# yukyeongleee/pggan

Hardware: AMD Instinct MI355X
Metric: images/sec (G+D+GP step) at 1024×1024 bs=4/GPU, 1/2/4/8 MI355X (higher is better)
Workload: dtype bf16; 1 GPU; C5 G+D+R1 train_step via ProgressiveGAN.train_step, stage 8 (1024x1024), batch 4/GPU, alpha 1.0, depths [512, 512, 512, 512, 256, 128, 64, 32, 16] (alpha = 1: the fade-in's zero-weight low-resolution branches elided, results bit-identical on the CPU double, PG_ENGINE=elide_zero_blend=0 computes them); global_batch=4, resolution=1024, parallelism=dp1

## Files before the change

### include/pggan_hip.h

```cpp
#ifndef PGGAN_HIP_H
#define PGGAN_HIP_H
#include <stddef.h>
#include <stdint.h>

#ifdef __cplusplus
extern "C" {
#endif

#define PG_OK 0
#define PG_ERR_ARG (-1)
#define PG_ERR_HIP (-2)
#define PG_ERR_UNSUPPORTED (-3)

#define PG_F32 0
#define PG_BF16 1

const char* pg_last_error(void);
int pg_version(void);

#define PG_SCRATCH_BYTES (4u << 20)
size_t pg_scratch_bytes(void);

#define PG_CONV_UPS_IN 1
#define PG_CONV_BIAS 2
#define PG_CONV_LRELU 4
#define PG_CONV_MASK 8
#define PG_CONV_POOL 16
#define PG_CONV_ACCUM 32
#define PG_CONV_PIXNORM 64
#define PG_CONV_Y2_BITS 128
#define PG_CONV_AUX_BITS 256
#define PG_CONV_X_BITS 512
#define PG_CONV_GZ_BITS 1024
#define PG_CONV_PNBWD 2048
#define PG_CONV_RGBW 4096
#define PG_CONV_RGBD 8192
#define PG_CONV_RGBO 16384

typedef struct {
  int B, H, W;
  int cin, cout;
  int x_cs, y_cs, aux_cs, y2_cs;
  int flags;
  float slope;
  float out_scale;
  int xb_cs;
} pg_conv_desc;

#define PG_PACK_FWD 0
#define PG_PACK_DGRAD 1
size_t pg_conv3x3_packed_elems(int mode, int cout, int cin);
int pg_conv3x3_pack(int dtype, int mode, int cout, int cin, const float* w_oihw, float scale,
                    void* wpk, void* stream);
typedef struct {
  const float* w;
  const float* bias;
  void* fwd;
  void* dgrad;
  float* bias_scaled;
  float scale;
  int cout, cin;
  int pad_;
} pg_pack_item;
int pg_conv3x3_pack_batch(int dtype, int n, const pg_pack_item* items, int max_tiles,
                          void* stream);
size_t pg_conv3x3_workspace_size(const pg_conv_desc* d);
int pg_conv3x3_fwd(int dtype, const pg_conv_desc* d, const void* x, const void* wpk,
                   const float* bias, const void* aux, void* y, void* y2, void* ws,
                   size_t ws_bytes, void* stream);
int pg_conv3x3_fwd_ex(int dtype, const pg_conv_desc* d, const void* x, const void* xbits,
                      const void* wpk, const float* bias, const void* aux, void* y, void* y2,
                      void* ws, size_t ws_bytes, void* stream);
int pg_conv3x3_rgbw(int dtype, const pg_conv_desc* d, const void* x, const void* wpk,
                    const void* aux, const float* img, float s, float* dw, float* db,
                    void* scratch, void* stream);
int pg_conv3x3_rgbd(int dtype, const pg_conv_desc* d, const void* x, const void* wpk,
                    const void* aux, const float* w_rgb, float f, float* gimg, float* norms,
                    float* dw, float s, void* scratch, void* stream);
int pg_conv3x3_rgbo(int dtype, const pg_conv_desc* d, const void* x, const void* wpk,
                    const float* bias, void* y, void* y2, const float* w_rgb, const float* b_rgb,
                    float c, float* img, void* stream);
int pg_conv3x3_supported(int dtype, const pg_conv_desc* d, size_t ws_bytes);
size_t pg_conv3x3_wgrad_workspace_size(int dtype, const pg_conv_desc* d);
int pg_conv3x3_wgrad(int dtype, const pg_conv_desc* d, const void* x, const void* gz, float scale,
                     float* dw, float* db, void* ws, size_t ws_bytes, void* stream);
int pg_conv3x3_wgrad_ex(int dtype, const pg_conv_desc* d, const void* x, const void* gz,
                        const void* gzbits, float scale, float* dw, float* db, void* ws,
                        size_t ws_bytes, void* stream);
int pg_bias_grad(int dtype, int npix, int C, int cs, const void* g, float scale, float* db,
                 void* scratch, void* stream);

int pg_pixnorm_fwd(int dtype, int npix, int C, int cs, const void* x, void* y, void* stream);
int pg_pixnorm_lrelu_bwd(int dtype, int npix, int C, int cs, const void* u, const void* gy,
                         float slope, int apply_mask, void* gz, void* stream);

int pg_pixnorm_lrelu_bwd_y(int dtype, int npix, int C, int cs, const void* y, const float* r,
                           const void* gy, float slope, void* gz, void* stream);
int pg_unpool_mask(int dtype, int B, int H, int W, int C, int g_cs, const void* g, int y_cs,
                   const void* y, float scale, float slope, int ups, int out_cs, void* out,
                   void* stream);
int pg_unpool_mask_bits(int dtype, int B, int H, int W, int C, int g_cs, const void* g,
                        const void* bits, float scale, float slope, int ups, int out_cs, void* out,
                        void* stream);
int pg_avgpool2(int dtype, int B, int H, int W, int C, int x_cs, const void* x, int y_cs, void* y,
                void* stream);
int pg_blend(int dtype, size_t n, float a, const void* x, float b, const void* y, void* out,
             void* stream);

int pg_rgb_out(int dtype, int B, int R, int C, int x_cs, const void* x, const float* w,
               const float* b, float c, int Cp, int xp_cs, const void* xp, const float* wp,
               const float* bp, float cp, float alpha, float* img, void* stream);
int pg_rgb_out_bwd(int dtype, int B, int R, int C, int x_cs, const void* x, const float* w,
                   float c, int Cp, int xp_cs, const void* xp, const float* wp, float cp,
                   float alpha, const float* gimg, void* gx, void* gxp, float* dw, float* db,
                   float* dwp, float* dbp, void* scratch, void* stream);
int pg_rgb_out_bwd_pn(int dtype, int B, int R, int C, int y_cs, const void* y, const float* r,
                      const float* w, float c, const float* gimg, float slope, int gz_cs, void* gz,
                      void* stream);
int pg_rgb_out_bwd_pn_wg(int dtype, int B, int R, int C, int y_cs, const void* y, const float* r,
                         const float* w, float c, const float* gimg, float slope, int gz_cs,
                         void* gz, float* dw, float* db, void* scratch, void* stream);
int pg_from_rgb(int dtype, int B, int R, int C, const float* img, int down, const float* w,
                const float* b, float c, float slope, const void* mask_y, int y_cs, void* y,
                void* stream);
int pg_from_rgb_bwd(int dtype, int B, int R, int C, const float* img, int down, const float* w,
                    float c, int gz_cs, const void* gz, float* gimg, float* dw, float* db,
                    void* scratch, void* stream);
typedef struct {
  const float* x0;
  const float* x1;
  const float* a;
  const float* c;
} pg_img_src;
int pg_from_rgb_src(int dtype, int B, int R, int C, const pg_img_src* img, int down, const float* w,
                    const float* b, float c, float slope, const void* mask_y, int y_cs, void* y,
                    void* stream);
int pg_from_rgb_bits(int dtype, int B, int R, int C, const pg_img_src* img, int down,
                     const float* w, const float* b, float c, float slope, const void* mask_bits,
                     int y_cs, void* y, void* ybits, void* stream);
int pg_from_rgb_bwd_src(int dtype, int B, int R, int C, const pg_img_src* img, int down,
                        const float* w, float c, int gz_cs, const void* gz, float* gimg,
                        int gimg_overwrite, float* norms, float* dw, float* db, void* scratch,
                        void* stream);
int pg_penalty_scale(int mode, int B, float* norms, float w, float* loss_out, float* scale,
                     void* stream);

int pg_img_fade(int B, int C, int R, const float* x, float alpha, float* out, void* stream);

#define PG_LIN_BIAS 1
#define PG_LIN_LRELU 2
#define PG_LIN_MASK 4
#define PG_LIN_IN_CHW 8
#define PG_LIN_OUT_CHW 16
#define PG_LIN_F32_IN 32
#define PG_LIN_F32_OUT 64
typedef struct {
  int B, K, N;
  int in_cs, out_cs;
  int flags;
  float scale, slope;
} pg_linear_desc;
int pg_linear_fwd(int dtype, const pg_linear_desc* d, const void* x, const float* w,
                  const float* b, const void* aux, void* y, void* stream);
int pg_linear_dgrad(int dtype, const pg_linear_desc* d, const void* gy, const float* w,
                    const void* aux, void* gx, void* stream);
size_t pg_linear_workspace_size(int dtype, const pg_linear_desc* d, int pass);
int pg_linear_fwd_ws(int dtype, const pg_linear_desc* d, const void* x, const float* w,
                     const float* b, const void* aux, void* y, void* ws, size_t ws_bytes,
                     void* stream);
int pg_linear_dgrad_ws(int dtype, const pg_linear_desc* d, const void* gy, const float* w,
                       const void* aux, void* gx, void* ws, size_t ws_bytes, void* stream);
// ... 67 lines not shown
```

### pggan_amd/_lib.py

```python
from __future__ import annotations

import ctypes
import os

import torch

PG_F32, PG_BF16 = 0, 1

CONV_UPS_IN, CONV_BIAS, CONV_LRELU, CONV_MASK, CONV_POOL, CONV_ACCUM = 1, 2, 4, 8, 16, 32
CONV_PIXNORM = 64
CONV_PNBWD = 2048
CONV_RGBW = 4096
CONV_RGBD = 8192
CONV_RGBO = 16384
CONV_Y2_BITS, CONV_AUX_BITS, CONV_X_BITS, CONV_GZ_BITS = 128, 256, 512, 1024
PACK_FWD, PACK_DGRAD = 0, 1
LIN_BIAS, LIN_LRELU, LIN_MASK, LIN_IN_CHW, LIN_OUT_CHW, LIN_F32_IN, LIN_F32_OUT = (
    1, 2, 4, 8, 16, 32, 64)

_HERE = os.path.dirname(os.path.abspath(__file__))
LIB_PATH = os.path.join(_HERE, "libpggan_hip.so")


class ConvDesc(ctypes.Structure):
    _fields_ = [(n, ctypes.c_int) for n in
                ("B", "H", "W", "cin", "cout", "x_cs", "y_cs", "aux_cs", "y2_cs", "flags")] + \
               [("slope", ctypes.c_float), ("out_scale", ctypes.c_float), ("xb_cs", ctypes.c_int)]


class PackItem(ctypes.Structure):
    _fields_ = [("w", ctypes.c_void_p), ("bias", ctypes.c_void_p), ("fwd", ctypes.c_void_p),
                ("dgrad", ctypes.c_void_p), ("bias_scaled", ctypes.c_void_p),
                ("scale", ctypes.c_float), ("cout", ctypes.c_int), ("cin", ctypes.c_int),
                ("pad_", ctypes.c_int)]


def _cinp(c):
    return (c + 7) // 8 * 8 if c <= 16 else (c + 31) // 32 * 32


class ImgMix:

    def __init__(self, x0, x1=None, a=None, c=None):
        self.x0, self.x1, self.a, self.c = x0, x1, a, c

    @property
    def shape(self):
        return self.x0.shape

    @property
    def device(self):
        return self.x0.device

    def materialize(self):
        if self.a is None:
            return self.x0
        v = self.a.view(-1, 1, 1, 1) * self.x0
        if self.x1 is not None:
            v = v + self.c.view(-1, 1, 1, 1) * self.x1
        return v


class ImgSrcDesc(ctypes.Structure):
    _fields_ = [("x0", ctypes.c_void_p), ("x1", ctypes.c_void_p), ("a", ctypes.c_void_p),
                ("c", ctypes.c_void_p)]


class LinearDesc(ctypes.Structure):
    _fields_ = [(n, ctypes.c_int) for n in ("B", "K", "N", "in_cs", "out_cs", "flags")] + \
               [("scale", ctypes.c_float), ("slope", ctypes.c_float)]


_lib = None
_SIDE_STREAMS = {}

_VP, _I, _F, _SZ, _U64 = ctypes.c_void_p, ctypes.c_int, ctypes.c_float, ctypes.c_size_t, ctypes.c_uint64
_SIGS = {
    "pg_version": ([], _I),
    "pg_scratch_bytes": ([], _SZ),
    "pg_conv3x3_packed_elems": ([_I, _I, _I], _SZ),
    "pg_conv3x3_pack": ([_I, _I, _I, _I, _VP, _F, _VP, _VP], _I),
    "pg_conv3x3_pack_batch": ([_I, _I, _VP, _I, _VP], _I),
    "pg_conv3x3_workspace_size": ([ctypes.POINTER(ConvDesc)], _SZ),
    "pg_conv3x3_fwd": ([_I, ctypes.POINTER(ConvDesc), _VP, _VP, _VP, _VP, _VP, _VP, _VP, _SZ, _VP],
                       _I),
    "pg_conv3x3_supported": ([_I, ctypes.POINTER(ConvDesc), _SZ], _I),
    "pg_conv3x3_rgbw": ([_I, ctypes.POINTER(ConvDesc), _VP, _VP, _VP, _VP, _F, _VP, _VP, _VP, _VP],
                        _I),
    "pg_conv3x3_rgbd": ([_I, ctypes.POINTER(ConvDesc), _VP, _VP, _VP, _VP, _F, _VP, _VP, _VP, _F,
                         _VP, _VP], _I),
    "pg_conv3x3_rgbo": ([_I, ctypes.POINTER(ConvDesc), _VP, _VP, _VP, _VP, _VP, _VP, _VP, _F, _VP,
                         _VP], _I),
    "pg_conv3x3_fwd_ex": ([_I, ctypes.POINTER(ConvDesc), _VP, _VP, _VP, _VP, _VP, _VP, _VP, _VP,
                           _SZ, _VP], _I),
    "pg_conv3x3_wgrad_ex": ([_I, ctypes.POINTER(ConvDesc), _VP, _VP, _VP, _F, _VP, _VP, _VP, _SZ,
                             _VP], _I),
    "pg_conv3x3_wgrad_workspace_size": ([_I, ctypes.POINTER(ConvDesc)], _SZ),
    "pg_conv3x3_wgrad": ([_I, ctypes.POINTER(ConvDesc), _VP, _VP, _F, _VP, _VP, _VP, _SZ, _VP],
                         _I),
    "pg_bias_grad": ([_I, _I, _I, _I, _VP, _F, _VP, _VP, _VP], _I),
    "pg_pixnorm_fwd": ([_I, _I, _I, _I, _VP, _VP, _VP], _I),
    "pg_pixnorm_lrelu_bwd": ([_I, _I, _I, _I, _VP, _VP, _F, _I, _VP, _VP], _I),
    "pg_pixnorm_lrelu_bwd_y": ([_I, _I, _I, _I, _VP, _VP, _VP, _F, _VP, _VP], _I),
    "pg_unpool_mask": ([_I, _I, _I, _I, _I, _I, _VP, _I, _VP, _F, _F, _I, _I, _VP, _VP], _I),
    "pg_unpool_mask_bits": ([_I, _I, _I, _I, _I, _I, _VP, _VP, _F, _F, _I, _I, _VP, _VP], _I),
    "pg_avgpool2": ([_I, _I, _I, _I, _I, _I, _VP, _I, _VP, _VP], _I),
    "pg_blend": ([_I, _SZ, _F, _VP, _F, _VP, _VP, _VP], _I),
    "pg_rgb_out": ([_I, _I, _I, _I, _I, _VP, _VP, _VP, _F, _I, _I, _VP, _VP, _VP, _F, _F, _VP,
                    _VP], _I),
    "pg_rgb_out_bwd": ([_I, _I, _I, _I, _I, _VP, _VP, _F, _I, _I, _VP, _VP, _F, _F, _VP, _VP,
                        _VP, _VP, _VP, _VP, _VP, _VP, _VP], _I),
    "pg_from_rgb": ([_I, _I, _I, _I, _VP, _I, _VP, _VP, _F, _F, _VP, _I, _VP, _VP], _I),
    "pg_from_rgb_bwd": ([_I, _I, _I, _I, _VP, _I, _VP, _F, _I, _VP, _VP, _VP, _VP, _VP, _VP], _I),
    "pg_img_fade": ([_I, _I, _I, _VP, _F, _VP, _VP], _I),
    "pg_from_rgb_src": ([_I, _I, _I, _I, ctypes.POINTER(ImgSrcDesc), _I, _VP, _VP, _F, _F, _VP, _I,
                         _VP, _VP], _I),
    "pg_rgb_out_bwd_pn": ([_I, _I, _I, _I, _I, _VP, _VP, _VP, _F, _VP, _F, _I, _VP, _VP], _I),
    "pg_rgb_out_bwd_pn_wg": ([_I, _I, _I, _I, _I, _VP, _VP, _VP, _F, _VP, _F, _I, _VP, _VP, _VP,
                              _VP, _VP], _I),
    "pg_from_rgb_bits": ([_I, _I, _I, _I, ctypes.POINTER(ImgSrcDesc), _I, _VP, _VP, _F, _F, _VP,
                          _I, _VP, _VP, _VP], _I),
    "pg_from_rgb_bwd_src": ([_I, _I, _I, _I, ctypes.POINTER(ImgSrcDesc), _I, _VP, _F, _I, _VP, _VP,
                             _I, _VP, _VP, _VP, _VP, _VP], _I),
    "pg_penalty_scale": ([_I, _I, _VP, _F, _VP, _VP, _VP], _I),
    "pg_linear_fwd": ([_I, ctypes.POINTER(LinearDesc), _VP, _VP, _VP, _VP, _VP, _VP], _I),
    "pg_linear_dgrad": ([_I, ctypes.POINTER(LinearDesc), _VP, _VP, _VP, _VP, _VP], _I),
    "pg_linear_wgrad": ([_I, ctypes.POINTER(LinearDesc), _VP, _VP, _VP, _VP, _VP], _I),
    "pg_linear_workspace_size": ([_I, ctypes.POINTER(LinearDesc), _I], _SZ),
    "pg_linear_fwd_ws": ([_I, ctypes.POINTER(LinearDesc), _VP, _VP, _VP, _VP, _VP, _VP, _SZ, _VP],
                         _I),
    "pg_linear_dgrad_ws": ([_I, ctypes.POINTER(LinearDesc), _VP, _VP, _VP, _VP, _VP, _SZ, _VP],
                           _I),
    "pg_mbstd_fwd": ([_I, _I, _I, _I, _I, _VP, _I, _VP, _VP], _I),
    "pg_mbstd_bwd": ([_I, _I, _I, _I, _I, _VP, _I, _VP, _VP, _VP], _I),
    "pg_mbstd_r1": ([_I, _I, _I, _I, _I, _VP, _VP, _I, _VP, _VP, _VP, _VP], _I),
    "pg_bce_loss": ([_I, _VP, _I, _F, _VP, _VP, _VP, _VP], _I),
    "pg_r1_penalty": ([_I, _SZ, _VP, _VP, _VP, _VP, _VP], _I),
    "pg_drift_loss": ([_I, _VP, _F, _VP, _VP, _VP], _I),
    "pg_gp_interp": ([_I, _SZ, _VP, _VP, _VP, _VP, _VP], _I),
    "pg_gp_penalty": ([_I, _SZ, _VP, _F, _VP, _VP, _VP, _VP, _VP], _I),
    "pg_mul_add": ([_SZ, _VP, _VP, _VP, _VP, _VP], _I),
    "pg_adam": ([_SZ, _VP, _VP, _VP, _VP, _F, _F, _F, _F, _I, _VP], _I),
    "pg_randn": ([_SZ, _U64, _U64, _VP, _VP], _I),
    "pg_randn_dev": ([_SZ, _U64, _VP, _VP, _VP], _I),
    "pg_adam_table_len": ([_F, _F, _F], _I),
    "pg_adam_table": ([_F, _F, _F, _I, _VP], _I),
    "pg_adam_dev": ([_SZ, _VP, _VP, _VP, _VP, _F, _F, _F, _VP, _I, _VP, _VP], _I),
    "pg_cast": ([_I, _I, _SZ, _VP, _VP, _VP], _I),
    "pg_augment_workspace_bytes": ([_I, _I, _I], _SZ),
    "pg_augment_u8": ([_I, _I, _I, _VP, _VP, _VP, _SZ, _VP, _VP], _I),
    "pg_step_plan_create": ([_I, _I, ctypes.POINTER(ctypes.c_int), _I, _I,
                             ctypes.POINTER(ctypes.c_void_p)], _I),
    "pg_step_plan_workspace_size": ([_VP], _SZ),
    "pg_step_plan_describe": ([_VP, ctypes.c_char_p, _SZ], _I),
    "pg_step_plan_destroy": ([_VP], None),
    "pg_event_create": ([_I, ctypes.POINTER(ctypes.c_void_p)], _I),
    "pg_event_record": ([_VP, _VP], _I),
    "pg_stream_wait_event": ([_VP, _VP], _I),
    "pg_event_elapsed_ms": ([_VP, _VP, ctypes.POINTER(ctypes.c_float)], _I),
    "pg_event_destroy": ([_VP], _I),
    "pg_fill_zero": ([_VP, _SZ, _VP], _I),
    "pg_copy": ([_VP, _VP, _SZ, _VP], _I),
    "pg_record_begin": ([], _I),
    "pg_record_end": ([ctypes.POINTER(ctypes.c_void_p)], _I),
    "pg_record_count": ([_VP], _I),
    "pg_replay": ([_VP], _I),
    "pg_record_destroy": ([_VP], None),
    "pg_stream_create": ([_I, ctypes.POINTER(ctypes.c_void_p)], _I),
    "pg_stream_destroy": ([_VP], _I),
}
SYMBOLS = ["pg_last_error"] + list(_SIGS)


def load_library(path: str = LIB_PATH):
    global _lib
    if _lib is not None:
        return _lib
    if not os.path.exists(path):
        raise RuntimeError(f"pggan_amd: HIP library not built: {path} (run __graft_entry__.build())")
    lib = ctypes.CDLL(path)
    lib.pg_last_error.argtypes = []
    lib.pg_last_error.restype = ctypes.c_char_p
# ... 152 lines not shown
    def conv_pack(self, mode, w, scale, out):
        self._cuda(w, out)
        cout, cin = w.shape[0], w.shape[1]
        self._chk(self.lib.pg_conv3x3_pack(self._dt(out), mode, cout, cin, _p(w), scale, _p(out),
                                           self._s()), "conv3x3_pack")

    def pack_table(self, entries):
        n = len(entries)
        arr = (PackItem * n)()
        mt = 1
        for i, (w, b, pf, pd, bs, sc) in enumerate(entries):
            self._cuda(w, b, pf, pd, bs)
            cout, cin = w.shape[0], w.shape[1]
            arr[i] = PackItem(_p(w), _p(b), _p(pf), _p(pd), _p(bs), float(sc), cout, cin, 0)
            O = max((cout + 15) // 16 * 16, _cinp(cout))
            C = max(_cinp(cin), (cin + 15) // 16 * 16)
            mt = max(mt, ((O + 31) // 32) * ((C + 31) // 32))
        raw = torch.frombuffer(bytearray(bytes(arr)), dtype=torch.uint8)
        return raw.to(entries[0][0].device), n, mt

    def conv_pack_batch(self, table):
        dev, n, mt = table
        self._cuda(dev)
        self._chk(self.lib.pg_conv3x3_pack_batch(self.dt, n, _p(dev), mt, self._s()),
                  "conv3x3_pack_batch")

    def conv3x3(self, x, wpk, y, *, B, H, W, cin, cout, flags, slope=0.2, out_scale=1.0,
                bias=None, aux=None, y2=None, ws=None, xbits=None):
        self._cuda(x, wpk, y, bias, aux, y2, ws, xbits)
        d = ConvDesc(B, H, W, cin, cout, x.shape[-1], y.shape[-1],
                     aux.shape[-1] if aux is not None else 0,
                     y2.shape[-1] if y2 is not None else 0, flags, slope, out_scale,
                     xbits.shape[-1] if xbits is not None else 0)
        wsb = ws.numel() * ws.element_size() if ws is not None else 0
        self._chk(self.lib.pg_conv3x3_fwd_ex(self._dt(y), ctypes.byref(d), _p(x), _p(xbits),
                                             _p(wpk), _p(bias), _p(aux), _p(y), _p(y2), _p(ws),
                                             wsb, self._s()),
                  "conv3x3_fwd")

    def conv3x3_rgbw(self, x, wpk, *, B, H, W, cin, cout, flags, aux, img, s, dw, db,
                     slope=0.2, out_scale=1.0):
        self._cuda(x, wpk, aux, img, dw, db)
        d = ConvDesc(B, H, W, cin, cout, x.shape[-1], cout, aux.shape[-1], 0,
                     flags | CONV_RGBW, slope, out_scale, 0)
        self._chk(self.lib.pg_conv3x3_rgbw(self._dt(x), ctypes.byref(d), _p(x), _p(wpk), _p(aux),
                                           _p(img), float(s), _p(dw), _p(db),
                                           self._scr(), self._s()),
                  "conv3x3_rgbw")

    def conv3x3_rgbo(self, x, wpk, y, *, B, H, W, cin, cout, flags, bias, w_rgb, b_rgb, c, img,
                     y2=None, slope=0.2):
        self._cuda(x, wpk, y, bias, y2, w_rgb, b_rgb, img)
        d = ConvDesc(B, H, W, cin, cout, x.shape[-1], y.shape[-1], 0,
                     y2.shape[-1] if y2 is not None else 0, flags | CONV_RGBO, slope, 1.0, 0)
        self._chk(self.lib.pg_conv3x3_rgbo(self._dt(y), ctypes.byref(d), _p(x), _p(wpk), _p(bias),
                                           _p(y), _p(y2), _p(w_rgb), _p(b_rgb), float(c), _p(img),
                                           self._s()),
                  "conv3x3_rgbo")

    def conv3x3_rgbd(self, x, wpk, *, B, H, W, cin, cout, flags, aux, w_rgb, f, gimg,
                     norms=None, dw=None, s=0.0, slope=0.2, out_scale=1.0):
        self._cuda(x, wpk, aux, w_rgb, gimg, norms, dw)
        d = ConvDesc(B, H, W, cin, cout, x.shape[-1], cout, aux.shape[-1], 0,
                     flags | CONV_RGBD, slope, out_scale, 0)
        self._chk(self.lib.pg_conv3x3_rgbd(self._dt(x), ctypes.byref(d), _p(x), _p(wpk), _p(aux),
                                           _p(w_rgb), float(f), _p(gimg), _p(norms), _p(dw),
                                           float(s), self._scr(), self._s()),
                  "conv3x3_rgbd")

    def conv_supported(self, *, B, H, W, cin, cout, flags, ws_bytes=0):
        if flags & CONV_GZ_BITS:
            return self.dt == PG_BF16 and H % 2 == 0 and W % 2 == 0 and cout % 8 == 0
        d = ConvDesc(B, H, W, cin, cout, 0, 0, 0, 0, flags, 0.2, 1.0, 0)
        return bool(self.lib.pg_conv3x3_supported(self.dt, ctypes.byref(d), ws_bytes))

    def conv_workspace_bytes(self, *, B, H, W, cin, cout):
        d = ConvDesc(B, H, W, cin, cout, 0, 0, 0, 0, 0, 0.0, 1.0, 0)
        return int(self.lib.pg_conv3x3_workspace_size(ctypes.byref(d)))

    def wgrad_workspace_bytes(self, *, B, H, W, cin, cout, ups=False):
        d = ConvDesc(B, H, W, cin, cout, 0, 0, 0, 0, CONV_UPS_IN if ups else 0, 0.0, 1.0, 0)
        return int(self.lib.pg_conv3x3_wgrad_workspace_size(self.dt, ctypes.byref(d)))

    def conv_wgrad(self, x, gz, dw, *, B, H, W, cin, cout, ups, scale, db=None, ws=None,
                   gzbits=None, slope=0.2):
        self._cuda(x, gz, dw, db, ws, gzbits)
        fl = (CONV_UPS_IN if ups else 0) | (CONV_GZ_BITS if gzbits is not None else 0)
        d = ConvDesc(B, H, W, cin, cout, x.shape[-1], gz.shape[-1], 0, 0, fl, slope, 1.0,
                     gzbits.shape[-1] if gzbits is not None else 0)
        wsb = ws.numel() * ws.element_size() if ws is not None else 0
        self._chk(self.lib.pg_conv3x3_wgrad_ex(self._dt(gz), ctypes.byref(d), _p(x), _p(gz),
                                               _p(gzbits), scale, _p(dw), _p(db), _p(ws), wsb,
                                               self._s()),
                  "conv3x3_wgrad")

    def bias_grad(self, g, db, C, scale):
        self._cuda(g, db)
        npix = g.numel() // g.shape[-1]
        self._chk(self.lib.pg_bias_grad(self._dt(g), npix, C, g.shape[-1], _p(g), scale, _p(db),
                                        self._scr(), self._s()), "bias_grad")

    def pixnorm(self, x, y, C):
        self._cuda(x, y)
        npix = x.numel() // x.shape[-1]
        self._chk(self.lib.pg_pixnorm_fwd(self._dt(x), npix, C, x.shape[-1], _p(x), _p(y),
                                          self._s()), "pixnorm_fwd")

    def pixnorm_lrelu_bwd(self, u, gy, gz, C, slope, mask=True):
        self._cuda(u, gy, gz)
        npix = u.numel() // u.shape[-1]
        self._chk(self.lib.pg_pixnorm_lrelu_bwd(self._dt(u), npix, C, u.shape[-1], _p(u), _p(gy),
                                                slope, 1 if mask else 0, _p(gz), self._s()),
                  "pixnorm_lrelu_bwd")

    def pixnorm_lrelu_bwd_y(self, y, r, gy, gz, C, slope):
        self._cuda(y, r, gy, gz)
        npix = y.numel() // y.shape[-1]
        self._chk(self.lib.pg_pixnorm_lrelu_bwd_y(self._dt(y), npix, C, y.shape[-1], _p(y), _p(r),
                                                  _p(gy), slope, _p(gz), self._s()),
                  "pixnorm_lrelu_bwd_y")

    def unpool_mask(self, g, y, out, *, B, H, W, C, scale, slope, ups, bits=None):
        self._cuda(g, y, out, bits)
        if bits is not None:
            self._chk(self.lib.pg_unpool_mask_bits(self._dt(out), B, H, W, C, g.shape[-1], _p(g),
                                                   _p(bits), scale, slope, 1 if ups else 0,
                                                   out.shape[-1], _p(out), self._s()),
                      "unpool_mask_bits")
            return
        self._chk(self.lib.pg_unpool_mask(self._dt(out), B, H, W, C, g.shape[-1], _p(g),
                                          y.shape[-1] if y is not None else 0, _p(y), scale, slope,
                                          1 if ups else 0, out.shape[-1], _p(out), self._s()),
                  "unpool_mask")

    def avgpool2(self, x, y, *, B, H, W, C):
        self._cuda(x, y)
        self._chk(self.lib.pg_avgpool2(self._dt(x), B, H, W, C, x.shape[-1], _p(x), y.shape[-1],
                                       _p(y), self._s()), "avgpool2")

    def blend(self, a, x, b, y, out):
        self._cuda(x, y, out)
        self._chk(self.lib.pg_blend(self._dt(out), out.numel(), a, _p(x), b, _p(y), _p(out),
                                    self._s()), "blend")

    def rgb_out(self, x, w, b, c, img, *, B, R, C, xp=None, wp=None, bp=None, cp=0.0, Cp=0,
                alpha=1.0):
        self._cuda(x, w, b, img, xp, wp, bp)
        self._chk(self.lib.pg_rgb_out(self._dt(x), B, R, C, x.shape[-1], _p(x), _p(w), _p(b), c, Cp,
                                      xp.shape[-1] if xp is not None else 0, _p(xp), _p(wp), _p(bp),
                                      cp, alpha, _p(img), self._s()), "rgb_out")

    def rgb_out_bwd(self, x, w, c, gimg, gx, dw, db, *, B, R, C, xp=None, wp=None, cp=0.0, Cp=0,
                    alpha=1.0, gxp=None, dwp=None, dbp=None):
        self._cuda(x, w, gimg, gx, dw, db, xp, wp, gxp, dwp, dbp)
        self._chk(self.lib.pg_rgb_out_bwd(self._dt(x), B, R, C, x.shape[-1], _p(x), _p(w), c, Cp,
                                          xp.shape[-1] if xp is not None else 0, _p(xp), _p(wp), cp,
                                          alpha, _p(gimg), _p(gx), _p(gxp), _p(dw), _p(db), _p(dwp),
                                          _p(dbp), self._scr(), self._s()), "rgb_out_bwd")

    def rgb_out_bwd_pn(self, y, r, w, c, gimg, gz, *, B, R, C, slope, dw=None, db=None):
        if dw is not None:
            self._cuda(y, r, w, gimg, gz, dw, db)
            self._chk(self.lib.pg_rgb_out_bwd_pn_wg(self._dt(y), B, R, C, y.shape[-1], _p(y), _p(r),
                                                    _p(w), c, _p(gimg), slope, gz.shape[-1], _p(gz),
                                                    _p(dw), _p(db), self._scr(), self._s()),
                      "rgb_out_bwd_pn_wg")
            return
        self._cuda(y, r, w, gimg, gz)
        self._chk(self.lib.pg_rgb_out_bwd_pn(self._dt(y), B, R, C, y.shape[-1], _p(y), _p(r), _p(w), c,
                                             _p(gimg), slope, gz.shape[-1], _p(gz), self._s()),
                  "rgb_out_bwd_pn")

    def _src(self, img):
# ... 179 lines not shown
```

### pggan_amd/csrc/conv.hip

```cpp
#include <cstdarg>
#include <cstdio>
#include <cstdlib>
#include <type_traits>

#include "common.h"

namespace {

struct ConvParams {
  const void* x;
  const void* w;
  const float* bias;
  const void* aux;
  void* y;
  void* y2;
  int B, H, W, Hin, Win;
  int cin_p, cout, cout_p;
  int x_cs, y_cs, aux_cs, y2_cs;
  int flags;
  float slope, out_scale;
  int NB, TH, TW, tiles_x, tiles_y;
  int CK, KS, nchunks;
  int pixb, wrowb, halo_bytes;
  float* ws;
// ... 656 lines not shown
    __syncthreads();
    if (do_db)
      for (int pm = 0; pm < WG_BP; ++pm) bsum += gzl[pm * WG_RS + tid];
    for (int k0 = 0; k0 < WG_BP; k0 += 4) {
      const int pm = k0 + g;
      const int tx = pm % p.TW, ty = (pm / p.TW) % p.TH, nb = pm / (p.TW * p.TH);
      const int hbase = (nb * (p.TH + 2) + ty) * TW2 + tx;
      const float a = gzl[pm * WG_RS + om + r];
#pragma unroll
      for (int tap = 0; tap < 9; ++tap) {
        const float bb = hal[(hbase + (tap / 3) * TW2 + (tap % 3)) * WG_RS + cn + r];
        acc[tap] = __builtin_amdgcn_mfma_f32_16x16x4f32(a, bb, acc[tap], 0, 0, 0);
      }
    }
  }
  float* slab = p.ws ? p.ws + blockIdx.z * p.slab : nullptr;
  if (do_db && o0 + tid < p.cout) {
    if (slab) slab[(size_t)p.cout * p.cin * 9 + o0 + tid] = bsum;
    else p.db[o0 + tid] += bsum * p.scale;
  }
  const int c = cc0 + cn + r;
#pragma unroll
  for (int j = 0; j < 4; ++j) {
    const int o = o0 + om + 4 * g + j;
    if (o < p.cout && c < p.cin) {
      const size_t e = ((size_t)o * p.cin + c) * 9;
      if (slab) {
#pragma unroll
        for (int tap = 0; tap < 9; ++tap) slab[e + tap] = acc[tap][j];
      } else {
#pragma unroll
        for (int tap = 0; tap < 9; ++tap) p.dw[e + tap] += acc[tap][j] * p.scale;
      }
    }
  }
}

static int wgrad_f32_splits(const pg_conv_desc* d, int* tiles_per_split) {
  TileCfg tc = pick_tile(d->H, d->W, WG_BP, 32);
  const int ntiles = pg_cdiv(d->B, tc.NB) * (d->W / tc.TW) * (d->H / tc.TH);
  const int ot = pg_cdiv(d->cout, WG_BO), ct = pg_cdiv(d->cin, WG_BC);
  int splits = pg_cdiv(2048, ot * ct);
  if (splits > ntiles) splits = ntiles;
  if (splits < 1) splits = 1;
  *tiles_per_split = pg_cdiv(ntiles, splits);
  return pg_cdiv(ntiles, *tiles_per_split);
}
static size_t wgrad_f32_ws_bytes(const pg_conv_desc* d) {
  int tps;
  const int splits = wgrad_f32_splits(d, &tps);
  return splits > 1 ? (size_t)splits * ((size_t)d->cout * d->cin * 9 + d->cout) * sizeof(float) : 0;
}

typedef __attribute__((ext_vector_type(4))) __bf16 bf16x4_t;
typedef __attribute__((address_space(3))) bf16x4_t lds_bf16x4_t;

__device__ __forceinline__ bf16x8_t tr_read8(const bf16_t* lo, const bf16_t* hi) {
  bf16x4_t a = __builtin_amdgcn_ds_read_tr16_b64_v4bf16((lds_bf16x4_t*)lo);
  bf16x4_t b = __builtin_amdgcn_ds_read_tr16_b64_v4bf16((lds_bf16x4_t*)hi);
  return __builtin_shufflevector(a, b, 0, 1, 2, 3, 4, 5, 6, 7);
}

enum { WG_DIRECT = 0, WG_SLABS = 1 };

struct WgBParams {
  const bf16_t* x;
  const bf16_t* gz;
  float* dw;
  float* db;
  float* ws;
  size_t slab;
  int mode;
  int B, H, W, Hin, Win;
  int cin, cout, x_cs, gz_cs;
  int ups;
  float scale;
  int NB, TH, TW, tiles_x, tiles_y, ntiles, tiles_per_split;
  int GZS, HS, halo_elems, hpad;
  int lg_tx, lg_ty;
  const unsigned char* gzb;
  int gzb_cs;
  float slope;
  int xcd_remap;
};

constexpr int WGB_BP = 128;
constexpr int wgb_maxhalo(int bp) { return bp == 128 ? 288 : 18 * 18; }

__device__ __forceinline__ float bf_lo(unsigned u) { return __uint_as_float(u << 16); }
__device__ __forceinline__ float bf_hi(unsigned u) { return __uint_as_float(u & 0xffff0000u); }

#ifndef PG_WG_PRE_ALL
#define PG_WG_PRE_ALL 1
#endif
template <int MO, int NC, int WMO, int WNC, int PD, int WPE, bool GZB, int BP>
__global__ __launch_bounds__(256) __attribute__((amdgpu_waves_per_eu(WPE)))
void wgrad_bf16_kernel(WgBParams p) {
  constexpr bool PRE = PG_WG_PRE_ALL || MO < 4;
  constexpr int KW = 4 / (WMO * WNC);
  constexpr int BO = WMO * MO * 16, BC = WNC * NC * 16;
  constexpr int GV = BO / 8, HV = BC / 8;
  constexpr int NGZ = BP * GV / 256;
  constexpr int NH = (wgb_maxhalo(BP) * HV + 255) / 256;
  static_assert(NGZ * 256 == BP * GV, "gz staging must tile the workgroup");
  extern __shared__ __attribute__((aligned(16))) char smem[];
  bf16_t* gzl = reinterpret_cast<bf16_t*>(smem);
  constexpr int GZS = BO + (BO > 16 ? 16 : 0), HS = BC == 16 ? 16 : BC + 16;
  const int hpad = p.hpad;
  auto grow = [](int r) { return r * GZS + (r >> 3) * 64; };
  auto hrow = [hpad](int r) { return r * HS + (r >> 3) * hpad; };
  bf16_t* hal = gzl + grow(BP);
  const int hscr = hrow(p.halo_elems);
  const int tid = threadIdx.x, lane = tid & 63, wid = tid >> 6;
  const int wk = wid % KW, wmn = wid / KW;
  const int wo = wmn / WNC, wc = wmn % WNC;
  const int g = lane >> 4, i16 = lane & 15, q = i16 >> 2, pq = i16 & 3;
  int bx = blockIdx.x, by = blockIdx.y, bz = blockIdx.z;
  if (p.xcd_remap) {
    const int ox = gridDim.x, oy = gridDim.y;
    const int n = ox * oy * gridDim.z;
    const int h = bx + ox * (by + oy * bz);
    const int xcd = h & 7, slot = h >> 3, q = n >> 3, rr = n & 7;
    const int L = (xcd < rr ? xcd * (q + 1) : rr * (q + 1) + (xcd - rr) * q) + slot;
    bx = L % ox;
    by = (L / ox) % oy;
    bz = L / (ox * oy);
  }
  const int o0 = bx * BO, c0 = by * BC;
  const int TW2 = p.TW + 2, HW2 = (p.TH + 2) * TW2;
  const int nhalo = p.halo_elems * HV;

  f32x4_t acc[MO][NC][9];
#pragma unroll
  for (int a = 0; a < MO; ++a)
#pragma unroll
    for (int b = 0; b < NC; ++b)
#pragma unroll
      for (int t = 0; t < 9; ++t) acc[a][b][t] = f32x4_t{0.f, 0.f, 0.f, 0.f};

  const bool do_db = p.db && by == 0;
  float bs[8];
#pragma unroll
  for (int e = 0; e < 8; ++e) bs[e] = 0.f;

  constexpr bool gz_bits = GZB;
  const int gH = gz_bits ? p.H >> 1 : p.H, gW = gz_bits ? p.W >> 1 : p.W;
  int gzrel[NGZ], gznb[NGZ], hpk[NH], gbrel[NGZ], hrel[NH];
#pragma unroll
  for (int k = 0; k < NGZ; ++k) {
    const int i = tid + k * 256;
    const int pm = i / GV, v = i - pm * GV;
    const int tx = pm % p.TW, ty = (pm / p.TW) % p.TH, nb = pm / (p.TW * p.TH);
    const int gs = gz_bits ? 1 : 0;
    gzrel[k] = ((nb * gH + (ty >> gs)) * gW + (tx >> gs)) * p.gz_cs + 8 * v;
    gbrel[k] = ((nb * p.H + ty) * p.W + tx) * p.gzb_cs + ((o0 + 8 * v) >> 3);
    gznb[k] = (o0 + 8 * v < p.cout) ? nb : 1 << 20;
  }
#pragma unroll
  for (int k = 0; k < NH; ++k) {
    const int i = tid + k * 256;
    hpk[k] = -1;
    if (i < nhalo) {
      const int hp = i / HV, v = i - hp * HV;
      const int nb = hp / HW2, rem = hp - nb * HW2;
      const int hy = rem / TW2, hx = rem - hy * TW2;
      if (c0 + 8 * v < p.x_cs) hpk[k] = (nb << 24) | (hy << 16) | (hx << 8) | v;
    }
    const int pk = hpk[k] < 0 ? 0 : hpk[k];
    const int ys = p.ups ? 1 : 0;
    if constexpr (PRE) hrel[k] = (((pk >> 24) * p.Hin + ((((pk >> 16) & 0xff) - 1) >> ys)) * p.Win +
               ((((pk >> 8) & 0xff) - 1) >> ys)) * p.x_cs + 8 * (pk & 0xff);
  }
  auto load_tile = [&](int t, u32x4_t (&rg)[NGZ], u32x4_t (&rh)[NH], int (&rb)[NGZ],
                       unsigned& gok, unsigned& hok) {
    constexpr bool sh = PRE;
    const int tx0 = (sh && p.lg_tx >= 0 ? (t & (p.tiles_x - 1)) : t % p.tiles_x) * p.TW;
    const int tt = sh && p.lg_tx >= 0 ? t >> p.lg_tx : t / p.tiles_x;
    const int ty0 = (sh && p.lg_ty >= 0 ? (tt & (p.tiles_y - 1)) : tt % p.tiles_y) * p.TH;
    const int b0 = (sh && p.lg_ty >= 0 ? tt >> p.lg_ty : tt / p.tiles_y) * p.NB;
    const int gs = gz_bits ? 1 : 0;
    gok = 0;
    hok = 0;
    const bf16_t* gzt = p.gz + (((size_t)b0 * gH + (ty0 >> gs)) * gW + (tx0 >> gs)) * p.gz_cs + o0;
    const unsigned char* gbt =
        gz_bits ? p.gzb + (((size_t)b0 * p.H + ty0) * p.W + tx0) * p.gzb_cs : nullptr;
#pragma unroll
    for (int k = 0; k < NGZ; ++k) {
      const bool ok = b0 + gznb[k] < p.B;
      rg[k] = *reinterpret_cast<const u32x4_t*>(ok ? gzt + gzrel[k] : p.gz);
      if constexpr (gz_bits) rb[k] = *(ok ? gbt + gbrel[k] : p.gzb);
      gok |= (ok ? 1u : 0u) << k;
    }
    const int ys = p.ups ? 1 : 0;
    const bf16_t* xt = PRE ? p.x + c0 + (((size_t)b0 * p.Hin + (ty0 >> ys)) * p.Win + (tx0 >> ys)) * p.x_cs
                              : p.x;
#pragma unroll
    for (int k = 0; k < NH; ++k) {
      const int pk = hpk[k];
      const int yy = ty0 + ((pk >> 16) & 0xff) - 1, xx = tx0 + ((pk >> 8) & 0xff) - 1;
      const bool ok = pk >= 0 && b0 + (pk >> 24) < p.B && (unsigned)yy < (unsigned)p.H &&
                      (unsigned)xx < (unsigned)p.W;
      if constexpr (PRE) {
        rh[k] = *reinterpret_cast<const u32x4_t*>(ok ? xt + hrel[k] : p.x);
      } else {
        rh[k] = *reinterpret_cast<const u32x4_t*>(
            ok ? p.x + c0 + (((size_t)(b0 + (pk >> 24)) * p.Hin + (yy >> ys)) * p.Win + (xx >> ys)) * p.x_cs +
                     8 * (pk & 0xff)
               : p.x);
      }
      hok |= (ok ? 1u : 0u) << k;
    }
  };
  auto store_tile = [&](const u32x4_t (&rg0)[NGZ], const u32x4_t (&rh)[NH], const int (&rb)[NGZ],
                        unsigned gok, unsigned hok) {
#pragma unroll
    for (int k = 0; k < NGZ; ++k) {
      const int i = tid + k * 256;
      const int pm = i / GV, v = i - pm * GV;
      const bool ok = (gok >> k) & 1u;
      u32x4_t rg = ok ? rg0[k] : u32x4_t{0u, 0u, 0u, 0u};
      if (gz_bits && ok && rb[k] != 0xff) {
        const int m = rb[k];
#pragma unroll
        for (int e = 0; e < 4; ++e) {
          float a = bf_lo(rg[e]), c = bf_hi(rg[e]);
          if (!((m >> (2 * e)) & 1)) a *= p.slope;
          if (!((m >> (2 * e + 1)) & 1)) c *= p.slope;
          rg[e] = pack_bf16x2(a, c);
        }
      }
      *reinterpret_cast<u32x4_t*>(gzl + grow(pm) + 8 * v) = rg;
      if (do_db) {
#pragma unroll
        for (int e = 0; e < 4; ++e) {
          bs[2 * e] += bf_lo(rg[e]);
          bs[2 * e + 1] += bf_hi(rg[e]);
        }
      }
    }
#pragma unroll
    for (int k = 0; k < NH; ++k) {
      const int i = tid + k * 256;
      const int hp = i / HV, v = i - hp * HV;
      const int off = i < nhalo ? hrow(hp) + 8 * v : hscr;
      *reinterpret_cast<u32x4_t*>(hal + off) = ((hok >> k) & 1u) ? rh[k] : u32x4_t{0u, 0u, 0u, 0u};
    }
  };
  constexpr int KSW = (BP / 32) / KW;
  int hAo[KSW], hBo[KSW];
#pragma unroll
  for (int j = 0; j < KSW; ++j) {
    const int ks = wk + j * KW;
    const int rA = ks * 32 + 8 * g + q, rB = rA + 4;
    const int txA = rA % p.TW, tyA = (rA / p.TW) % p.TH, nbA = rA / (p.TW * p.TH);
    const int txB = rB % p.TW, tyB = (rB / p.TW) % p.TH, nbB = rB / (p.TW * p.TH);
    hAo[j] = (nbA * (p.TH + 2) + tyA) * TW2 + txA;
    hBo[j] = (nbB * (p.TH + 2) + tyB) * TW2 + txB;
  }
  auto compute_tile = [&]() {
#pragma unroll
    for (int j = 0; j < KSW; ++j) {
      const int ks = wk + j * KW;
      const int rA = ks * 32 + 8 * g + q, rB = rA + 4;
      bf16x8_t A[MO];
#pragma unroll
      for (int mo = 0; mo < MO; ++mo) {
        const int ol = (wo * MO + mo) * 16 + 4 * pq;
        A[mo] = tr_read8(gzl + grow(rA) + ol, gzl + grow(rB) + ol);
      }
      const int hA = hAo[j], hB = hBo[j];
      auto readB = [&](int tap, int nc) {
        const int toff = (tap / 3) * TW2 + (tap % 3);
        const int cl = (wc * NC + nc) * 16 + 4 * pq;
        return tr_read8(hal + hrow(hA + toff) + cl, hal + hrow(hB + toff) + cl);
      };
      bf16x8_t Bc = readB(0, 0);
#pragma unroll
      for (int tap = 0; tap < 9; ++tap) {
#pragma unroll
        for (int nc = 0; nc < NC; ++nc) {
          const bool last = tap == 8 && nc == NC - 1;
          const bf16x8_t Bn = last ? Bc : (nc + 1 < NC ? readB(tap, nc + 1) : readB(tap + 1, 0));
          if constexpr (MO >= 4) __builtin_amdgcn_sched_barrier(0);
#pragma unroll
          for (int mo = 0; mo < MO; ++mo)
            acc[mo][nc][tap] = __builtin_amdgcn_mfma_f32_16x16x32_bf16(A[mo], Bc, acc[mo][nc][tap],
                                                                       0, 0, 0);
          if constexpr (MO >= 4) __builtin_amdgcn_sched_barrier(0);
          Bc = Bn;
        }
      }
    }
  };

  u32x4_t rg[PD][NGZ], rh[PD][NH];
  int rb[PD][NGZ];
  unsigned gokr[PD], hokr[PD];
  const int t_begin = bz * p.tiles_per_split;
  const int t_end = min(p.ntiles, t_begin + p.tiles_per_split);
#pragma unroll
  for (int d = 0; d < PD; ++d)
    load_tile(min(t_begin + d, t_end - 1), rg[d], rh[d], rb[d], gokr[d], hokr[d]);
  for (int t = t_begin; t < t_end; t += PD) {
#pragma unroll
    for (int d = 0; d < PD; ++d) {
      const bool live = t + d < t_end;
      __syncthreads();
      store_tile(rg[d], rh[d], rb[d], live ? gokr[d] : 0u, live ? hokr[d] : 0u);
      __syncthreads();
      load_tile(min(t + d + PD, t_end - 1), rg[d], rh[d], rb[d], gokr[d], hokr[d]);
      if (live) compute_tile();
    }
  }

  float* red = reinterpret_cast<float*>(smem);
// ... 125 lines not shown
  float s[4] = {0.f, 0.f, 0.f, 0.f};
  for (int k = 0; k < splits; k += RSP) {
    f32x4_t t[RSP];
#pragma unroll
    for (int u = 0; u < RSP; ++u)
      if (k + u < splits) t[u] = *reinterpret_cast<const f32x4_t*>(ws + (size_t)(k + u) * slab + i);
#pragma unroll
    for (int u = 0; u < RSP; ++u)
      if (k + u < splits) {
#pragma unroll
        for (int e = 0; e < 4; ++e) s[e] += t[u][e];
      }
  }
  float* dst = i < (size_t)nw ? dw + i : (db ? db + (i - nw) : nullptr);
  if (!dst) return;
#pragma unroll
  for (int e = 0; e < 4; ++e) dst[e] += s[e] * scale;
}

struct WgbPlan {
  int MO, NC, WMO, WNC, BP;
  int ot, ct, splits, tiles_per_split, ntiles;
  TileCfg tc;
  size_t slab;
};

bool wgrad_dma_ok(const pg_conv_desc* d, const WgbPlan& pl);

WgbPlan wgrad_bf16_plan(const pg_conv_desc* d) {
  WgbPlan pl;
  const int co = d->cout, ci = d->cin;
  pl.MO = co <= 16 ? 1 : co <= 32 ? 2 : 4;
  pl.NC = 1;
  pl.WMO = 1;
  pl.WNC = ci <= 16 ? 1 : (ci <= 32 || d->W >= 32) ? 2 : 1;
  if (pl.WNC == 1 && ci > 16 && pg_cdiv(co, co <= 16 ? 16 : co <= 32 ? 32 : 64) * pg_cdiv(ci, 16) > 256)
    pl.WNC = 2;
  const int BO = pl.WMO * pl.MO * 16, BC = pl.WNC * pl.NC * 16;
  pl.BP = WGB_BP;
  pl.tc = pick_tile(d->H, d->W, pl.BP, 32);
  pl.ntiles = pg_cdiv(d->B, pl.tc.NB) * (d->W / pl.tc.TW) * (d->H / pl.tc.TH);
  pl.ot = pg_cdiv(co, BO);
  pl.ct = pg_cdiv(ci, BC);
  const int base = pl.ot * pl.ct;
  int target = pl.MO >= 4 ? 192 : 512;
  if (pl.MO < 4) {
    pl.tiles_per_split = 1;
    if (wgrad_dma_ok(d, pl)) {
      if (pl.MO == 2 && pl.WNC == 2) target = 256;
      else if (pl.MO == 1 && pl.WNC == 1) target = 1024;
    }
  }
  int splits = base >= 256 ? 1 : pg_cdiv(target, base);
  const int max_splits = pl.ntiles / 2 > 1 ? pl.ntiles / 2 : 1;
  if (splits > max_splits) splits = max_splits;
  if (splits < 1) splits = 1;
  pl.tiles_per_split = pg_cdiv(pl.ntiles, splits);
  pl.splits = pg_cdiv(pl.ntiles, pl.tiles_per_split);
  pl.slab = (size_t)co * ci * 9 + co;
  return pl;
}

size_t wgrad_bf16_ws_bytes(const pg_conv_desc* d) {
  WgbPlan pl = wgrad_bf16_plan(d);
  return pl.splits > 1 ? pl.splits * pl.slab * sizeof(float) : 0;
}

int wgrad_slab_finish(const pg_conv_desc* d, const WgbPlan& pl, int mode, const float* ws, float* dw,
                      float* db, float scale, hipStream_t st) {
  if (mode != WG_SLABS) return PG_OK;
  if (pl.slab >= 65536 && pl.slab % 4 == 0 && ((uintptr_t)ws & 15) == 0) {
    PG_KLAUNCH(wgrad_slab_reduce4, dim3((unsigned)pg_cdiv((long long)pl.slab / 4, 64)), dim3(64), 0, st,
                       ws, pl.slab, pl.splits, d->cout * d->cin * 9, dw, db, scale);
    PG_LAUNCH_CHECK();
    return PG_OK;
  }
  launch_slab_reduce(ws, pl.slab, pl.splits, d->cout * d->cin * 9, dw, db, scale, st);
  PG_LAUNCH_CHECK();
  return PG_OK;
}

bool wgrad_dma_ok(const pg_conv_desc* d, const WgbPlan& pl);
int launch_wgrad_dma(const pg_conv_desc* d, const WgbPlan& pl, const void* x, const void* gz, float scale,
                     float* dw, float* db, float* ws, size_t ws_bytes, hipStream_t st, const void* gzbits);

template <int MO, int NC, int WMO, int WNC, int PD, int WPE, bool GZB = false, int BP = WGB_BP>
int launch_wgrad_bf16(const pg_conv_desc* d, const WgbPlan& pl, const void* x, const void* gz,
                      float scale, float* dw, float* db, float* ws, size_t ws_bytes,
                      hipStream_t st, const void* gzbits) {
  constexpr int BO = WMO * MO * 16, BC = WNC * NC * 16;
  WgBParams p;
  p.x = (const bf16_t*)x; p.gz = (const bf16_t*)gz; p.dw = dw; p.db = db;
  p.B = d->B; p.H = d->H; p.W = d->W;
  p.ups = (d->flags & PG_CONV_UPS_IN) ? 1 : 0;
  p.Hin = p.ups ? d->H / 2 : d->H;
  p.Win = p.ups ? d->W / 2 : d->W;
  p.cin = d->cin; p.cout = d->cout; p.x_cs = d->x_cs; p.gz_cs = d->y_cs;
  p.scale = scale;
  p.NB = pl.tc.NB; p.TH = pl.tc.TH; p.TW = pl.tc.TW;
  p.tiles_x = d->W / pl.tc.TW;
  p.tiles_y = d->H / pl.tc.TH;
  auto lg2 = [](int v) { int l = 0; while ((1 << l) < v) ++l; return (1 << l) == v ? l : -1; };
  p.lg_tx = lg2(p.tiles_x);
  p.lg_ty = lg2(p.tiles_y);
  p.ntiles = pl.ntiles;
  p.tiles_per_split = pl.tiles_per_split;
  p.GZS = BO + (BO > 16 ? 16 : 0);
  p.HS = BC == 16 ? 16 : BC + 16;
  p.hpad = pl.tc.TW >= 8 ? 64 : 0;
  p.halo_elems = pl.tc.NB * (pl.tc.TH + 2) * (pl.tc.TW + 2);
  p.gzb = (d->flags & PG_CONV_GZ_BITS) ? reinterpret_cast<const unsigned char*>(gzbits) : nullptr;
  p.gzb_cs = d->xb_cs;
  p.slope = d->slope;
  p.xcd_remap = 1;
  PG_CHECK_ARG(!p.gzb || (d->xb_cs * 8 >= d->cout && pl.tc.TH % 2 == 0 && pl.tc.TW % 2 == 0),
               "wgrad_bf16: GZ_BITS needs gzbits with >= cout/8 bytes per pixel");
  PG_CHECK_ARG(pl.BP == BP && p.halo_elems <= wgb_maxhalo(BP), "wgrad_bf16: halo %d > %d", p.halo_elems,
               wgb_maxhalo(BP));
  p.slab = pl.slab;
  p.ws = nullptr;
  PG_CHECK_ARG(pl.splits == 1 || (ws && ws_bytes >= pl.splits * pl.slab * sizeof(float)),
               "wgrad: split plan without its workspace");
  p.mode = pl.splits == 1 ? WG_DIRECT : WG_SLABS;
  if (p.mode == WG_SLABS) p.ws = ws;
  int lds = (BP * p.GZS + (BP / 8) * 64 + p.halo_elems * p.HS + (p.halo_elems / 8 + 1) * p.hpad) * 2 + 16;
  const int need = 4 * 9 * 64 * 4 * 4;
  if (need > lds) lds = need;
  PG_CHECK_ARG(lds <= 160 * 1024, "wgrad_bf16: LDS %d too large", lds);
  PG_LDS_ATTR((wgrad_bf16_kernel<MO, NC, WMO, WNC, PD, WPE, GZB, BP>), 160 * 1024);
  PG_KLAUNCH((wgrad_bf16_kernel<MO, NC, WMO, WNC, PD, WPE, GZB, BP>), dim3(pl.ot, pl.ct, pl.splits),
                     dim3(256), lds, st, p);
  PG_LAUNCH_CHECK();
  return wgrad_slab_finish(d, pl, p.mode, ws, dw, db, scale, st);
}

constexpr bool wgrad_gzb_ok(int MO, int WNC, int PD, int WPE) {
  return (MO == 2 && WNC == 1 && PD == 2 && WPE == 2) || (MO == 4 && PD == 4 && WPE == 1) ||
         (MO == 1 && PD == 2);
}

int wgrad_bf16_dispatch(const pg_conv_desc* d, const void* x, const void* gz, float scale,
                        float* dw, float* db, float* ws, size_t ws_bytes, hipStream_t st,
                        const void* gzbits = nullptr) {
  PG_CHECK_ARG(!(d->flags & PG_CONV_GZ_BITS) || gzbits, "wgrad_bf16: GZ_BITS without gzbits");
  PG_CHECK_ARG(d->cout % 8 == 0 && d->x_cs % 8 == 0 && d->y_cs % 8 == 0,
               "wgrad_bf16: cout (%d) and channel strides must be multiples of 8", d->cout);
  WgbPlan pl = wgrad_bf16_plan(d);
  if (pl.splits > 1 && !(ws && ws_bytes >= pl.splits * pl.slab * sizeof(float))) {
    pl.splits = 1;
    pl.tiles_per_split = pl.ntiles;
  }
  if (wgrad_dma_ok(d, pl)) return launch_wgrad_dma(d, pl, x, gz, scale, dw, db, ws, ws_bytes, st, gzbits);
  const int pd = pl.MO >= 4 ? 4 : 2, wpe = pl.MO >= 4 ? 1 : (pl.MO * pl.WNC >= 2 ? 2 : 3);
  const bool gzb = (d->flags & PG_CONV_GZ_BITS) != 0;
#define PG_WGB(a, b, c, e, PD, WPE)                                                        \
  if (pl.MO == a && pl.NC == b && pl.WMO == c && pl.WNC == e && pd == PD && wpe == WPE) {  \
    if constexpr (wgrad_gzb_ok(a, e, PD, WPE)) {                                           \
      if (gzb)                                                                             \
        return launch_wgrad_bf16<a, b, c, e, PD, WPE, true>(d, pl, x, gz, scale, dw, db,   \
                                                            ws, ws_bytes, st, gzbits);     \
    }                                                                                      \
    PG_CHECK_ARG(!gzb, "wgrad_bf16: GZ_BITS not instantiated for this tile");              \
    return launch_wgrad_bf16<a, b, c, e, PD, WPE, false>(d, pl, x, gz, scale, dw, db, ws,  \
                                                         ws_bytes, st, gzbits);            \
  }
  PG_WGB(1, 1, 1, 1, 2, 3)
  PG_WGB(1, 1, 1, 2, 2, 2)
  PG_WGB(2, 1, 1, 1, 2, 2)
  PG_WGB(2, 1, 1, 2, 2, 2)
  PG_WGB(4, 1, 1, 1, 4, 1)
  PG_WGB(4, 1, 1, 2, 4, 1)
#undef PG_WGB
  PG_CHECK_ARG(false, "wgrad_bf16: no kernel for plan");
  return PG_ERR_ARG;
}

template <typename T>
__global__ void pack_kernel(int mode, int cout, int cin, int rows, int kin, const float* w,
                            float scale, T* out) {
  const size_t total = (size_t)rows * 9 * kin;
  for (size_t i = blockIdx.x * (size_t)blockDim.x + threadIdx.x; i < total;
       i += (size_t)gridDim.x * blockDim.x) {
    const int k = (int)(i % kin);
    const int tap = (int)((i / kin) % 9);
    const int row = (int)(i / ((size_t)kin * 9));
    float v = 0.f;
    if (mode == PG_PACK_FWD) {
      if (row < cout && k < cin) v = w[((size_t)row * cin + k) * 9 + tap] * scale;
    } else {
      if (row < cin && k < cout) v = w[((size_t)k * cin + row) * 9 + (8 - tap)] * scale;
    }
    Ty<T>::st(out + i, v);
  }
}

template <typename T>
__global__ __launch_bounds__(256) void pack_batch_kernel(const pg_pack_item* items) {
  const pg_pack_item it = items[blockIdx.y];
  const int cout = it.cout, cin = it.cin;
  const int rf = (cout + 15) & ~15, kf = cinp_of_dev(cin);
  const int rd = (cin + 15) & ~15, kd = cinp_of_dev(cout);
  const int O = rf > kd ? rf : kd, C = kf > rd ? kf : rd;
  const int tc = (C + 31) / 32;
  if ((int)blockIdx.x >= ((O + 31) / 32) * tc) return;
  const int o0 = (blockIdx.x / tc) * 32, c0 = (blockIdx.x % tc) * 32;
  __shared__ float s[32][32 * 9 + 1];
  const int tid = threadIdx.x;
  if ((cin & 3) == 0 && ((uintptr_t)it.w & 15) == 0) {
#pragma unroll 3
    for (int i = tid; i < 32 * 72; i += 256) {
      const int ol = i / 72, j = (i - ol * 72) * 4;
      const int o = o0 + ol;
      f32x4_t v = f32x4_t{0.f, 0.f, 0.f, 0.f};
      if (o < cout && c0 + j / 9 < cin)
        v = *reinterpret_cast<const f32x4_t*>(it.w + ((size_t)o * cin + c0) * 9 + j);
#pragma unroll
      for (int k = 0; k < 4; ++k) s[ol][j + k] = (c0 + (j + k) / 9 < cin) ? v[k] * it.scale : 0.f;
    }
  } else {
    for (int i = tid; i < 32 * 288; i += 256) {
      const int ol = i / 288, j = i - ol * 288;
      const int o = o0 + ol, c = c0 + j / 9;
      s[ol][j] = (o < cout && c < cin) ? it.w[((size_t)o * cin + c0) * 9 + j] * it.scale : 0.f;
    }
  }
  __syncthreads();
  T* fwd = reinterpret_cast<T*>(it.fwd);
  T* dg = reinterpret_cast<T*>(it.dgrad);
  for (int i = tid; i < 8 * 288; i += 256) {
    const int cq = i & 7, tap = (i >> 3) % 9, ol = i / 72;
    const int o = o0 + ol, c = c0 + 4 * cq;
    float v[4];
#pragma unroll
    for (int k = 0; k < 4; ++k) v[k] = s[ol][(4 * cq + k) * 9 + tap];
    if (o < rf && c < kf) Ty<T>::st4(fwd + ((size_t)o * 9 + tap) * kf + c, v);
  }
  for (int i = tid; i < 8 * 288; i += 256) {
    const int oq = i & 7, tap = (i >> 3) % 9, cl = i / 72;
    const int o = o0 + 4 * oq, c = c0 + cl;
    float v[4];
#pragma unroll
    for (int k = 0; k < 4; ++k) v[k] = s[4 * oq + k][cl * 9 + 8 - tap];
    if (c < rd && o < kd) Ty<T>::st4(dg + ((size_t)c * 9 + tap) * kd + o, v);
  }
  if (c0 == 0 && tid < 32 && o0 + tid < cout)
// ... 354 lines not shown
  PG_CHECK_ARG(d->x_cs >= cinp_of(d->cin) && d->x_cs % 8 == 0 && d->aux_cs * 8 >= d->cout,
               "conv3x3_rgbd: bad channel strides");
  PG_CHECK_ARG(pg_det_fits((size_t)256 * 8, (size_t)16 + d->cout * 4), "conv3x3_rgbd: scratch too small");
  g_rgbw = RgbwArgs{};
  g_rgbw.rw = w_rgb; g_rgbw.f = f; g_rgbw.gimg = gimg; g_rgbw.norms = norms; g_rgbw.dw = dw;
  g_rgbw.s = s; g_rgbw.scratch = (float*)scratch;
  const int rc = conv_dispatch<bf16_t>(d, x, wpk, nullptr, aux, nullptr, nullptr, nullptr, 0,
                                       (hipStream_t)stream);
  g_rgbw = RgbwArgs{};
  return rc;
}

int pg_conv3x3_rgbo(int dtype, const pg_conv_desc* d, const void* x, const void* wpk,
                    const float* bias, void* y, void* y2, const float* w_rgb, const float* b_rgb,
                    float c, float* img, void* stream) {
  PG_CHECK_ARG(d && x && wpk && bias && y && w_rgb && b_rgb && img, "conv3x3_rgbo: null pointer");
  PG_CHECK_ARG(dtype == PG_BF16 && (d->flags & PG_CONV_RGBO) && conv_supported<bf16_t>(d, 0),
               "conv3x3_rgbo: flags 0x%x not supported for %d -> %d at %dx%d", d->flags, d->cin,
               d->cout, d->H, d->W);
  PG_CHECK_ARG(d->x_cs >= cinp_of(d->cin) && d->x_cs % 8 == 0 && d->y_cs >= d->cout,
               "conv3x3_rgbo: bad channel strides");
  g_rgbw = RgbwArgs{};
  g_rgbw.rw = w_rgb; g_rgbw.rb = b_rgb; g_rgbw.f = c; g_rgbw.gimg = img;
  const int rc = conv_dispatch<bf16_t>(d, x, wpk, bias, nullptr, y, y2, nullptr, 0,
                                       (hipStream_t)stream);
  g_rgbw = RgbwArgs{};
  return rc;
}

int pg_conv3x3_supported(int dtype, const pg_conv_desc* d, size_t ws_bytes) {
  if (!d) return 0;
  return (dtype == PG_F32 ? conv_supported<float>(d, ws_bytes) : conv_supported<bf16_t>(d, ws_bytes))
             ? 1 : 0;
}

size_t pg_conv3x3_wgrad_workspace_size(int dtype, const pg_conv_desc* d) {
  if (!d) return 0;
  return dtype == PG_BF16 ? wgrad_bf16_ws_bytes(d) : wgrad_f32_ws_bytes(d);
}

int pg_conv3x3_wgrad(int dtype, const pg_conv_desc* d, const void* x, const void* gz, float scale,
                     float* dw, float* db, void* ws, size_t ws_bytes, void* stream) {
  PG_CHECK_ARG(d && x && gz && dw, "conv3x3_wgrad: null pointer");
  PG_CHECK_ARG(d->B > 0 && d->H >= 4 && d->W >= 4, "conv3x3_wgrad: bad spatial size");
  PG_CHECK_ARG(!(d->flags & PG_CONV_GZ_BITS), "conv3x3_wgrad: GZ_BITS needs pg_conv3x3_wgrad_ex");
  if (dtype == PG_BF16)
    return wgrad_bf16_dispatch(d, x, gz, scale, dw, db, (float*)ws, ws_bytes, (hipStream_t)stream);
  TileCfg tc = pick_tile(d->H, d->W, WG_BP, 32);
  WgParams p;
  p.x = x; p.gz = gz; p.dw = dw; p.db = db;
  p.B = d->B; p.H = d->H; p.W = d->W;
  p.ups = (d->flags & PG_CONV_UPS_IN) ? 1 : 0;
  p.Hin = p.ups ? d->H / 2 : d->H;
  p.Win = p.ups ? d->W / 2 : d->W;
  p.cin = d->cin; p.cout = d->cout; p.x_cs = d->x_cs; p.gz_cs = d->y_cs;
  p.scale = scale;
  p.NB = tc.NB; p.TH = tc.TH; p.TW = tc.TW;
  p.tiles_x = d->W / tc.TW;
  p.tiles_y = d->H / tc.TH;
  p.ntiles = pg_cdiv(d->B, tc.NB) * p.tiles_x * p.tiles_y;
  const int ot = pg_cdiv(d->cout, WG_BO), ct = pg_cdiv(d->cin, WG_BC);
  int splits = wgrad_f32_splits(d, &p.tiles_per_split);
  p.slab = (size_t)d->cout * d->cin * 9 + d->cout;
  p.ws = nullptr;
  if (splits > 1 && ws && ws_bytes >= splits * p.slab * sizeof(float)) {
    p.ws = (float*)ws;
  } else {
    splits = 1;
    p.tiles_per_split = p.ntiles;
  }
  const int lds = (WG_BP * WG_RS + tc.NB * (tc.TH + 2) * (tc.TW + 2) * WG_RS) * 4;
  hipStream_t st = (hipStream_t)stream;
  dim3 grid(ot, ct, splits);
  if (dtype == PG_F32)
    PG_KLAUNCH(wgrad3x3_kernel<float>, grid, dim3(256), lds, st, p);
  else
    PG_KLAUNCH(wgrad3x3_kernel<bf16_t>, grid, dim3(256), lds, st, p);
  if (p.ws)
    launch_slab_reduce(p.ws, p.slab, splits, d->cout * d->cin * 9, dw, db, scale, st);
  PG_LAUNCH_CHECK();
  return PG_OK;
}

int pg_conv3x3_wgrad_ex(int dtype, const pg_conv_desc* d, const void* x, const void* gz,
                        const void* gzbits, float scale, float* dw, float* db, void* ws,
                        size_t ws_bytes, void* stream) {
  if (!d || !(d->flags & PG_CONV_GZ_BITS))
    return pg_conv3x3_wgrad(dtype, d, x, gz, scale, dw, db, ws, ws_bytes, stream);
  PG_CHECK_ARG(x && gz && gzbits && dw && dtype == PG_BF16, "conv3x3_wgrad_ex: GZ_BITS needs gzbits (bf16)");
  PG_CHECK_ARG(d->B > 0 && d->H >= 4 && d->W >= 4 && d->H % 2 == 0 && d->W % 2 == 0,
               "conv3x3_wgrad_ex: bad spatial size");
  return wgrad_bf16_dispatch(d, x, gz, scale, dw, db, (float*)ws, ws_bytes, (hipStream_t)stream,
                             gzbits);
}

int pg_bias_grad(int dtype, int npix, int C, int cs, const void* g, float scale, float* db,
                 void* scratch, void* stream) {
  PG_CHECK_ARG(g && db && npix > 0 && C > 0 && C <= 1024 && cs >= C && scratch,
               "bias_grad: bad args (C <= 1024, scratch required)");
  int ppb = 256;
  int blocks = pg_cdiv(npix, ppb);
  int cap = (int)(pg_scratch_floats() / (size_t)C);
  if (cap > 2048) cap = 2048;
  if (blocks > cap) {
    blocks = cap;
    ppb = pg_cdiv(npix, blocks);
    blocks = pg_cdiv(npix, ppb);
  }
  hipStream_t st = (hipStream_t)stream;
  if (dtype == PG_F32)
    PG_KLAUNCH(bias_grad_kernel<float>, dim3(blocks), dim3(256), 0, st, npix, C, cs,
                       (const float*)g, scale, db, ppb, (float*)scratch);
  else
    PG_KLAUNCH(bias_grad_kernel<bf16_t>, dim3(blocks), dim3(256), 0, st, npix, C, cs,
                       (const bf16_t*)g, scale, db, ppb, (float*)scratch);
  PG_LAUNCH_CHECK();
  return PG_OK;
}

}

namespace {
struct PlanLayer {
  char net, kind[8];
  int H, cin, cout, ups;
  int fwd_path, dgrad_path;
  int fwd_tile, dgrad_tile;
  size_t fwd_ws, dgrad_ws, wgrad_ws;
  int wg_MO, wg_WNC, wg_splits;
};
}

struct pg_step_plan {
  int dtype, stage, batch;
  size_t ws_bytes;
  int n;
  PlanLayer layers[64];
};

namespace {
void plan_conv(int dtype, pg_conv_desc* d, int* path, int* tile, size_t* ws) {
  *ws = conv_ws_bytes(d);
  *path = 0;
  *tile = -1;
  if (dtype == PG_BF16) {
    if (conv_lr_ok(d)) { *path = 2; *ws = 0; return; }
    if (conv_hr_ok(d)) { *path = 1; *tile = conv_hr_tile(d); *ws = 0; }
  }
}
}

extern "C" {

int pg_step_plan_create(int dtype, int n_depths, const int* depths, int stage, int batch,
                        pg_step_plan** out) {
  PG_CHECK_ARG(out && depths && stage >= 0 && stage + 1 <= n_depths && batch > 0 &&
                   (dtype == PG_F32 || dtype == PG_BF16),
               "step_plan_create: bad arguments");
  pg_step_plan* p = new pg_step_plan();
  p->dtype = dtype; p->stage = stage; p->batch = batch; p->ws_bytes = 0; p->n = 0;
  auto add = [&](char net, const char* kind, int H, int cin, int cout, int ups) {
    PlanLayer& L = p->layers[p->n++];
    L.net = net;
    snprintf(L.kind, sizeof(L.kind), "%s", kind);
    L.H = H; L.cin = cin; L.cout = cout; L.ups = ups;
    pg_conv_desc d{};
// ... 61 lines not shown
```

### pggan_amd/csrc/wgrad_dma.inc

```

constexpr int WGD_TH = 8, WGD_TW = 16, WGD_BP = WGD_TH * WGD_TW;
constexpr int WGD_HPIX = (WGD_TH + 2) * (WGD_TW + 2);
#ifndef PG_WGD_NSLOT
#define PG_WGD_NSLOT 4
#endif

template <int MO, int WNC, bool GZB = false>
struct WgdGeo {
  static constexpr int NW = 4 * WNC, NTHR = 64 * NW, KW = 4;
  static constexpr int GRB = 32 * MO, HPB = 32 * WNC;
  static constexpr int GP = WGD_BP * GRB / 1024;
  static constexpr int HP = (WGD_HPIX * HPB + 1023) / 1024;
  static constexpr int NPC = (GP + HP + NW - 1) / NW * NW;
  static constexpr int PPW = NPC / NW;
  static constexpr int GPW = GP / NW;
  static constexpr int BITS = GZB ? GP * 256 : 0;
  static constexpr int SLOT = NPC * 1024 + BITS;
  static constexpr int RED = NW * 2304 * 4;
  static constexpr int NSLOT = MO == 1 ? 3 : PG_WGD_NSLOT;
  static_assert(NSLOT >= 3 && NSLOT <= 4, "wgrad_dma: ring of 3-4 slots");
  static constexpr int LDS = NSLOT * SLOT > RED ? NSLOT * SLOT : RED;
};

template <int RB>
__device__ __forceinline__ int wgd_pos(int r) { return RB == 32 ? r ^ (((r >> 3) & 1) << 2) : r; }
template <int RB>
__device__ __forceinline__ int wgd_swz(int r) {
  return RB == 128 ? ((r & 2) | ((r & 8) >> 1)) : RB == 64 ? ((r >> 3) & 1) * 2 : 0;
}

__device__ __forceinline__ void wgd_dma4(const void* base, unsigned nrec, lds_void_t* dst, unsigned voff) {
  const size_t a = (size_t)base;
  const unsigned alo = __builtin_amdgcn_readfirstlane((unsigned)a);
  const unsigned ahi = __builtin_amdgcn_readfirstlane((unsigned)(a >> 32));
  const __amdgpu_buffer_rsrc_t rs = __builtin_amdgcn_make_buffer_rsrc(
      (void*)(((size_t)ahi << 32) | alo), 0, __builtin_amdgcn_readfirstlane(nrec), 0x00020000);
  const unsigned m0v = __builtin_amdgcn_readfirstlane((unsigned)(size_t)dst);
  unsigned keep;
  asm volatile("s_mov_b32 %0, m0\n\ts_mov_b32 m0, %1\n\tbuffer_load_dword %2, %3, 0 offen lds\n\t"
               "s_mov_b32 m0, %0"
               : "=&s"(keep) : "s"(m0v), "v"(voff), "s"(rs) : "memory");
}

template <int MO, int WNC, bool GZB>
__global__ __launch_bounds__(256 * WNC) void wgrad_dma_kernel(WgBParams p) {
#if defined(__HIP_DEVICE_COMPILE__)
  using G = WgdGeo<MO, WNC, GZB>;
  static_assert(!GZB || (G::GP % G::NW == 0 && MO >= 2), "wgrad_dma: GZB needs whole gz pieces per wave");
  constexpr int NW = G::NW, NTHR = G::NTHR, KW = G::KW, GRB = G::GRB, HPB = G::HPB;
  constexpr int BO = 16 * MO, BC = 16 * WNC;
  extern __shared__ __attribute__((aligned(16))) char smem[];
  const int tid = threadIdx.x, lane = tid & 63;
  const int wid = __builtin_amdgcn_readfirstlane(tid >> 6);
  const int wk = wid % KW, wc = wid / KW;
  const int g = lane >> 4, i16 = lane & 15, q = i16 >> 2, pq = i16 & 3;
  int bx = blockIdx.x, by = blockIdx.y, bz = blockIdx.z;
  if (p.xcd_remap) {
    const int ox = gridDim.x, oy = gridDim.y;
    const int n = ox * oy * gridDim.z;
    const int h = bx + ox * (by + oy * bz);
    const int xcd = h & 7, slot = h >> 3, qq = n >> 3, rr = n & 7;
    const int Lg = (xcd < rr ? xcd * (qq + 1) : rr * (qq + 1) + (xcd - rr) * qq) + slot;
    bx = Lg % ox;
    by = (Lg / ox) % oy;
    bz = Lg / (ox * oy);
  }
  const int o0 = bx * BO, c0 = by * BC;
  const bool do_db = p.db && by == 0;

  const unsigned OOB = 0x7fff0000u;
  const int gH = GZB ? p.H >> 1 : p.H, gW = GZB ? p.W >> 1 : p.W;
  const unsigned gz_nrec = (unsigned)((size_t)p.B * gH * gW * p.gz_cs * 2);
  const unsigned gzb_nrec = GZB ? (unsigned)((size_t)p.B * p.H * p.W * p.gzb_cs) : 0u;
  constexpr int PPP = 1024 / GRB;
  const unsigned x_nrec = (unsigned)((size_t)p.B * p.Hin * p.Win * p.x_cs * 2);
  const int ys = p.ups ? 1 : 0;
  auto dma_tile = [&](int t, char* base) __attribute__((always_inline)) {
    const int tx0 = (t & (p.tiles_x - 1)) * WGD_TW;
    const int tt = t >> p.lg_tx;
    const int ty0 = (tt & (p.tiles_y - 1)) * WGD_TH;
    const int b = tt >> p.lg_ty;
#pragma unroll
    for (int j = 0; j < G::PPW; ++j) {
      const int k = wid + NW * j;
      if (k < G::GP) {
        constexpr int SPR = GRB / 16;
        const int pos = k * (1024 / GRB) + lane / SPR;
        const int r = wgd_pos<GRB>(pos), s = (lane % SPR) ^ wgd_swz<GRB>(r);
        const int py = ty0 + (r >> 4), px = tx0 + (r & 15);
        const int gy = GZB ? py >> 1 : py, gx = GZB ? px >> 1 : px;
        const unsigned v = (unsigned)((((b * gH + gy) * gW + gx) * p.gz_cs + o0 + 8 * s) * 2);
        hr_dma16(p.gz, gz_nrec, (lds_void_t*)(base + k * 1024), v, 0);
        if constexpr (GZB) {
          constexpr int DPP = BO / 32;
          const int pi = lane / DPP;
          unsigned vb = OOB;
          if (pi < PPP) {
            const int r2 = k * PPP + pi;
            const int qy = ty0 + (r2 >> 4), qx = tx0 + (r2 & 15);
            vb = (unsigned)(((b * p.H + qy) * p.W + qx) * p.gzb_cs + (o0 >> 3) + 4 * (lane % DPP));
          }
          wgd_dma4(p.gzb, gzb_nrec, (lds_void_t*)(base + G::NPC * 1024 + k * 256), vb);
        }
      } else {
        constexpr int SPP = HPB / 16;
        const int pos = (k - G::GP) * (1024 / HPB) + lane / SPP;
        const int P = wgd_pos<HPB>(pos), s = (lane % SPP) ^ wgd_swz<HPB>(P);
        const int hy = P / (WGD_TW + 2), hx = P - hy * (WGD_TW + 2);
        const int yy = ty0 + hy - 1, xx = tx0 + hx - 1;
        unsigned v = OOB;
        if (P < WGD_HPIX && (unsigned)yy < (unsigned)p.H && (unsigned)xx < (unsigned)p.W)
          v = (unsigned)((((b * p.Hin + (yy >> ys)) * p.Win + (xx >> ys)) * p.x_cs + c0 + 8 * s) * 2);
        hr_dma16(p.x, x_nrec, (lds_void_t*)(base + k * 1024), v, 0);
      }
    }
  };

  const int rA = wk * 32 + 8 * g + q, rB = rA + 4;
  auto off_gz = [&](int r, int ol) { return wgd_pos<GRB>(r) * GRB + 16 * ((ol >> 3) ^ wgd_swz<GRB>(r)) + 2 * (ol & 7); };
  constexpr int NA = GRB == 32 ? 2 : 1;
  int offA[MO][NA], offB[9][2];
#pragma unroll
  for (int mo = 0; mo < MO; ++mo) {
    const int ol = mo * 16 + 4 * pq;
    offA[mo][0] = off_gz(rA, ol);
    if constexpr (NA == 2) offA[mo][NA - 1] = off_gz(rB, ol);
  }
  {
    const int cl = wc * 16 + 4 * pq;
    const int hA = (rA >> 4) * (WGD_TW + 2) + (rA & 15), hB = (rB >> 4) * (WGD_TW + 2) + (rB & 15);
#pragma unroll
    for (int tap = 0; tap < 9; ++tap) {
      const int toff = (tap / 3) * (WGD_TW + 2) + (tap % 3);
      const int PA = hA + toff, PB = hB + toff;
      offB[tap][0] = G::GP * 1024 + wgd_pos<HPB>(PA) * HPB + 16 * ((cl >> 3) ^ wgd_swz<HPB>(PA)) + 2 * (cl & 7);
      offB[tap][1] = G::GP * 1024 + wgd_pos<HPB>(PB) * HPB + 16 * ((cl >> 3) ^ wgd_swz<HPB>(PB)) + 2 * (cl & 7);
    }
  }

  f32x4_t acc[MO][9];
#pragma unroll
  for (int a = 0; a < MO; ++a)
#pragma unroll
    for (int t = 0; t < 9; ++t) acc[a][t] = f32x4_t{0.f, 0.f, 0.f, 0.f};
  float bs[8];
#pragma unroll
  for (int e = 0; e < 8; ++e) bs[e] = 0.f;

  auto compute = [&](const char* sb) __attribute__((always_inline)) {
    bf16x8_t A[MO];
#pragma unroll
    for (int mo = 0; mo < MO; ++mo)
      A[mo] = tr_read8(reinterpret_cast<const bf16_t*>(sb + offA[mo][0]),
                       reinterpret_cast<const bf16_t*>(sb + (NA == 2 ? offA[mo][NA - 1] : offA[mo][0] + 4 * GRB)));
    bf16x8_t Bc = tr_read8(reinterpret_cast<const bf16_t*>(sb + offB[0][0]),
                           reinterpret_cast<const bf16_t*>(sb + offB[0][1]));
#pragma unroll
    for (int tap = 0; tap < 9; ++tap) {
      const bf16x8_t Bn = tap + 1 < 9 ? tr_read8(reinterpret_cast<const bf16_t*>(sb + offB[tap + 1][0]),
                                                 reinterpret_cast<const bf16_t*>(sb + offB[tap + 1][1]))
                                      : Bc;
#pragma unroll
      for (int mo = 0; mo < MO; ++mo)
        acc[mo][tap] = __builtin_amdgcn_mfma_f32_16x16x32_bf16(A[mo], Bc, acc[mo][tap], 0, 0, 0);
      Bc = Bn;
    }
  };
  constexpr int GV = BO / 8;
  auto bias_tile = [&](const char* sb) __attribute__((always_inline)) {
#pragma unroll
    for (int j = 0; j < (WGD_BP * GV + NTHR - 1) / NTHR; ++j) {
      const int idx = tid + NTHR * j;
      if ((WGD_BP * GV) % NTHR != 0 && idx >= WGD_BP * GV) break;
      const int r = idx / GV, v = idx % GV;
      const u32x4_t u = *reinterpret_cast<const u32x4_t*>(
          sb + wgd_pos<GRB>(r) * GRB + 16 * (v ^ wgd_swz<GRB>(r)));
#pragma unroll
      for (int e = 0; e < 4; ++e) {
        bs[2 * e] += bf_lo(u[e]);
        bs[2 * e + 1] += bf_hi(u[e]);
      }
    }
  };

  const int t_begin = bz * p.tiles_per_split;
  const int t_end = min(p.ntiles, t_begin + p.tiles_per_split);
  const int n = t_end - t_begin;
  auto slot = [&](int i) -> char* { return smem + (i % G::NSLOT) * G::SLOT; };
  auto mask_tile = [&](char* sb) __attribute__((always_inline)) {
    constexpr int SPR = GRB / 16;
#pragma unroll
    for (int j = 0; j < G::GPW; ++j) {
      const int k = wid + NW * j;
      const int pos = k * PPP + lane / SPR;
      const int s = (lane % SPR) ^ wgd_swz<GRB>(pos);
      const int m = *reinterpret_cast<const unsigned char*>(sb + G::NPC * 1024 + k * 256 + (lane / SPR) * (BO / 8) + s);
      u32x4_t* q = reinterpret_cast<u32x4_t*>(sb + k * 1024 + lane * 16);
      *q = lrelu_mask_bf16x8(*q, (unsigned)m, p.slope);
    }
  };
  constexpr int OPT = G::PPW + (GZB ? G::GPW : 0);
  constexpr int DEPTH = G::NSLOT - 1;
#pragma unroll
  for (int d = 0; d < DEPTH; ++d)
    if (d < n) dma_tile(t_begin + d, slot(d));
  for (int i = 0; i < n; ++i) {
    const int younger = min(DEPTH - 1, n - 1 - i);
    if (younger >= 3) asm volatile("s_waitcnt vmcnt(%0)" ::"n"(3 * OPT) : "memory");
    else if (younger == 2) asm volatile("s_waitcnt vmcnt(%0)" ::"n"(2 * OPT) : "memory");
    else if (younger == 1) asm volatile("s_waitcnt vmcnt(%0)" ::"n"(OPT) : "memory");
    else asm volatile("s_waitcnt vmcnt(0)" ::: "memory");
    if constexpr (GZB) mask_tile(slot(i));
    asm volatile("s_waitcnt lgkmcnt(0)" ::: "memory");
    __builtin_amdgcn_s_barrier();
    asm volatile("" ::: "memory");
    if (i + DEPTH < n) dma_tile(t_begin + i + DEPTH, slot(i + DEPTH));
    compute(slot(i));
    if (do_db) bias_tile(slot(i));
  }

  float* red = reinterpret_cast<float*>(smem);
  asm volatile("s_waitcnt vmcnt(0) lgkmcnt(0)" ::: "memory");
  __syncthreads();
  if (do_db) {
#pragma unroll
    for (int e = 0; e < 8; ++e) red[tid * 8 + e] = bs[e];
    __syncthreads();
    if (tid < BO && o0 + tid < p.cout) {
      const int v = tid >> 3, e = tid & 7;
      float s = 0.f;
      for (int r = v; r < NTHR; r += GV) s += red[r * 8 + e];
      const int o = o0 + tid;
      if (p.mode == WG_SLABS)
        p.ws[bz * p.slab + (size_t)p.cout * p.cin * 9 + o] = s;
      else
        atomicAdd(p.db + o, s * p.scale);
    }
  }
  float* slab = p.mode == WG_SLABS ? p.ws + bz * p.slab : nullptr;
#pragma unroll 1
  for (int a = 0; a < MO; ++a) {
    __syncthreads();
    float* mine = red + (size_t)wid * 2304 + ((lane >> 4) * 64 + (lane & 15)) * 9;
#pragma unroll
    for (int mo = 0; mo < MO; ++mo)
      if (mo == a) {
#pragma unroll
        for (int t = 0; t < 9; ++t)
#pragma unroll
          for (int j = 0; j < 4; ++j) mine[j * 16 * 9 + t] = acc[mo][t][j];
      }
    __syncthreads();
    constexpr int NOUT = WNC * 2304;
    constexpr int NPT = NOUT / NTHR;
    static_assert(NPT * NTHR == NOUT, "wgrad_dma: epilogue split");
    float v[NPT];
    int offs[NPT];
#pragma unroll
    for (int k2 = 0; k2 < NPT; ++k2) {
      const int e = tid + NTHR * k2;
      const int m = e / 2304, rem = e - m * 2304;
      const int ol = rem / 144, rem2 = rem - ol * 144;
      const int cl = rem2 / 9, tap = rem2 - cl * 9;
      float sum = 0.f;
#pragma unroll
      for (int k = 0; k < KW; ++k) sum += red[(size_t)(m * KW + k) * 2304 + rem];
      const int o = o0 + a * 16 + ol;
      const int c = c0 + m * 16 + cl;
      v[k2] = sum;
      offs[k2] = (o < p.cout && c < p.cin) ? (o * p.cin + c) * 9 + tap : -1;
    }
    if (p.mode == WG_DIRECT) {
#pragma unroll
      for (int k2 = 0; k2 < NPT; ++k2)
        if (offs[k2] >= 0) atomicAdd(p.dw + offs[k2], v[k2] * p.scale);
    } else {
#pragma unroll
      for (int k2 = 0; k2 < NPT; ++k2)
        if (offs[k2] >= 0) slab[offs[k2]] = v[k2];
    }
  }
#endif
}

bool wgrad_dma_ok(const pg_conv_desc* d, const WgbPlan& pl) {
  const bool gzb = (d->flags & PG_CONV_GZ_BITS) != 0;
  if (gzb && (!((pl.MO == 4 && pl.WNC == 2) || (pl.MO == 2 && pl.WNC == 1)) || d->xb_cs % 4 ||
              d->xb_cs * 8 < d->cout || d->H % 2 || d->W % 2))
    return false;
  if (pl.NC != 1 || pl.WMO != 1 || pl.BP != 128) return false;
  const bool pair = (pl.MO == 4 && pl.WNC == 2) ||
                    (pl.MO == 2 && pl.WNC == 1) || (pl.MO == 1 && pl.WNC == 1) ||
                    (pl.MO == 1 && pl.WNC == 2) || (pl.MO == 2 && pl.WNC == 2);
  if (!pair) return false;
  if (pl.tc.TW != WGD_TW || pl.tc.TH != WGD_TH || pl.tc.NB != 1) return false;
  if (d->cout % (16 * pl.MO) || d->cin % (16 * pl.WNC) || d->x_cs % 8 || d->y_cs % 8) return false;
  const int tx = d->W / WGD_TW, ty = d->H / WGD_TH;
  if ((tx & (tx - 1)) || (ty & (ty - 1))) return false;
  const bool ups = (d->flags & PG_CONV_UPS_IN) != 0;
  const size_t xin = (size_t)d->B * (ups ? d->H / 2 : d->H) * (ups ? d->W / 2 : d->W) * d->x_cs * 2;
  const size_t gin = (size_t)d->B * (gzb ? d->H / 2 : d->H) * (gzb ? d->W / 2 : d->W) * d->y_cs * 2;
  const size_t bits = gzb ? (size_t)d->B * d->H * d->W * d->xb_cs : 0;
  return xin <= 0x7fff0000ull && gin <= 0x7fff0000ull && bits <= 0x7fff0000ull && pl.tiles_per_split >= 1;
}

template <int MO, int WNC, bool GZB = false>
int launch_wgrad_dma_k(const WgbPlan& pl, const WgBParams& p, hipStream_t st) {
  using G = WgdGeo<MO, WNC, GZB>;
  static_assert(G::NTHR * 8 * 4 <= G::LDS && G::LDS <= 160 * 1024, "wgrad_dma: LDS");
  PG_LDS_ATTR((wgrad_dma_kernel<MO, WNC, GZB>), G::LDS);
  PG_KLAUNCH((wgrad_dma_kernel<MO, WNC, GZB>), dim3(pl.ot, pl.ct, pl.splits), dim3(G::NTHR), G::LDS, st, p);
  PG_LAUNCH_CHECK();
  return PG_OK;
}

int launch_wgrad_dma(const pg_conv_desc* d, const WgbPlan& pl, const void* x, const void* gz, float scale,
                     float* dw, float* db, float* ws, size_t ws_bytes, hipStream_t st, const void* gzbits) {
  WgBParams p{};
  p.x = (const bf16_t*)x; p.gz = (const bf16_t*)gz; p.dw = dw; p.db = db;
  p.B = d->B; p.H = d->H; p.W = d->W;
  p.ups = (d->flags & PG_CONV_UPS_IN) ? 1 : 0;
  p.Hin = p.ups ? d->H / 2 : d->H;
  p.Win = p.ups ? d->W / 2 : d->W;
  p.cin = d->cin; p.cout = d->cout; p.x_cs = d->x_cs; p.gz_cs = d->y_cs;
  p.scale = scale;
  const bool gzb = (d->flags & PG_CONV_GZ_BITS) != 0;
  p.gzb = gzb ? reinterpret_cast<const unsigned char*>(gzbits) : nullptr;
  p.gzb_cs = d->xb_cs;
  p.slope = d->slope;
  PG_CHECK_ARG(!gzb || gzbits, "wgrad_dma: GZ_BITS without gzbits");
  p.tiles_x = d->W / WGD_TW;
  p.tiles_y = d->H / WGD_TH;
  auto lg2 = [](int v) { int l = 0; while ((1 << l) < v) ++l; return l; };
  p.lg_tx = lg2(p.tiles_x);
  p.lg_ty = lg2(p.tiles_y);
  p.ntiles = pl.ntiles;
  p.tiles_per_split = pl.tiles_per_split;
  p.xcd_remap = 1;
  p.slab = pl.slab;
  p.ws = nullptr;
  PG_CHECK_ARG(pl.splits == 1 || (ws && ws_bytes >= pl.splits * pl.slab * sizeof(float)),
               "wgrad: split plan without its workspace");
  p.mode = pl.splits == 1 ? WG_DIRECT : WG_SLABS;
  if (p.mode == WG_SLABS) p.ws = ws;
  PG_CHECK_ARG(pl.ntiles == d->B * p.tiles_x * p.tiles_y, "wgrad_dma: tile count");
  int rc;
  if (gzb && pl.MO == 4) rc = launch_wgrad_dma_k<4, 2, true>(pl, p, st);
  else if (gzb) rc = launch_wgrad_dma_k<2, 1, true>(pl, p, st);
  else if (pl.MO == 4) rc = launch_wgrad_dma_k<4, 2>(pl, p, st);
  else if (pl.MO == 2 && pl.WNC == 2) rc = launch_wgrad_dma_k<2, 2>(pl, p, st);
  else if (pl.MO == 2) rc = launch_wgrad_dma_k<2, 1>(pl, p, st);
  else if (pl.WNC == 2) rc = launch_wgrad_dma_k<1, 2>(pl, p, st);
  else rc = launch_wgrad_dma_k<1, 1>(pl, p, st);
  if (rc != PG_OK) return rc;
  return wgrad_slab_finish(d, pl, p.mode, ws, dw, db, scale, st);
}
```

### pggan_amd/engine.py

```python
from __future__ import annotations

import contextlib
import math
import os
from dataclasses import dataclass

import torch

from . import _lib as L

SLOPE = 0.2


def cinp(c):
    return ((c + 7) // 8) * 8 if c <= 16 else ((c + 31) // 32) * 32


def r4(c):
    return (c + 3) // 4 * 4


def he(fan_in):
    return math.sqrt(2.0 / fan_in)

# ... 46 lines not shown

class FlatParams:

    def __init__(self, shapes, dead, device, init=None):
        order = [n for n, _ in shapes if n not in dead] + [n for n, _ in shapes if n in dead]
        shp = dict(shapes)
        self.names = [n for n, _ in shapes]
        self.offsets, self.spans, off = {}, {}, 0
        self.n_live = 0
        for n in order:
            self.offsets[n] = off
            padded = (int(math.prod(shp[n])) + 15) // 16 * 16
            self.spans[n] = (off, off + padded)
            off += padded
            if n not in dead:
                self.n_live = off
        self.numel = off
        self.flat = torch.zeros(self.numel, dtype=torch.float32, device=device)
        self.grad = torch.zeros_like(self.flat)
        self.m = torch.zeros_like(self.flat)
        self.v = torch.zeros_like(self.flat)
        self.step = 0
        self.step_dev = torch.zeros(1, dtype=torch.int32, device=device)
        self._step_dev_host = 0
        self.shapes = shp
        self.dead = set(dead)
        self.views = {n: self._view(self.flat, n) for n in self.names}
        self.gviews = {n: self._view(self.grad, n) for n in self.names}
        if init is not None:
            for n in self.names:
                self.views[n].copy_(init[n])

    def _view(self, buf, n):
        o = self.offsets[n]
        return buf[o:o + int(math.prod(self.shapes[n]))].view(self.shapes[n])

    def live_grad(self):
        return self.grad[:self.n_live]

    def reset_optimizer(self):
        self.m.zero_()
        self.v.zero_()
        self.step = 0


@dataclass
class Hyper:
    lr_G: float = 1e-4
    lr_D: float = 1e-5
    beta1: float = 0.0
    beta2: float = 0.99
    eps: float = 1e-8
    W_adv: float = 1.0
    slope_cfg: float = 0.2
    gp_mode: str = "r1"
    W_gp: float = 10.0
    W_drift: float = 0.0


FORCE_SERIAL = False

ENGINE_DEFAULTS = dict(
    merge_d=True,
    merge_g=True,
    side_stream=True,
    elide_zero_blend=True,
    fuse_pixnorm=True,
    fuse_pnbwd=True,
    fuse_pn_pool=True,
    fuse_rgb_pnbwd=True,
    fuse_dbits=True,
    dbits_min_res=512,
    fuse_ubits=True,
    fuse_rgbbits=True,
    overlap_g_exchange=-1,
    tail_main=True,
    sep_b2=True,
    fuse_rgbw=True,
    fuse_rgbd=True,
    fuse_torgb_wg=True,
    tail_b=True,
    tail_levels=1,
    fuse_rgbo=False,
)


def engine_options(overrides=None):
    opts = dict(ENGINE_DEFAULTS)
    for item in filter(None, os.environ.get("PG_ENGINE", "").split(",")):
        k, _, v = item.partition("=")
        k = k.strip()
        if k not in opts:
            raise ValueError(f"PG_ENGINE: unknown option {k!r} (known: {sorted(opts)})")
        opts[k] = type(opts[k])(int(v)) if isinstance(opts[k], (bool, int)) else type(opts[k])(v)
    for k, v in (overrides or {}).items():
        if k not in opts:
            raise ValueError(f"unknown engine option {k!r}")
        opts[k] = v
    return opts


class StepEngine:

    def __init__(self, ops, depths, s, B, device, latent_dim=512, forward_only=None, **options):
        self.ops, self.depths, self.s, self.B = ops, list(depths), s, B
        self.forward_only = forward_only
        self.dev = device
        self.dt = ops.tdtype
        self.latent = latent_dim
        self.R = 4 * 2 ** s
        d = self.depths
        self.d0 = d[0]
        self.mcs = cinp(d[0] + 1)
        self.keep_fake_D = False
        for k, v in engine_options(options).items():
            setattr(self, k, v)
        self.ws = None
        self._ws_cache = {}
        self.plan = None
        if forward_only is None and hasattr(ops, "step_plan"):
            need, self.plan = ops.step_plan(self.depths, s, B)
            if need:
                self.ws = torch.empty((need + 3) // 4, dtype=torch.float32, device=device)
        self._last_dlow = True
        self.trace = None
        self.grad_ready = None
        self.side = None
        self._side_ev = {}
        self.ws_side = None
        if (forward_only is None and str(device).startswith("cuda") and self.side_stream and
                hasattr(ops, "side_stream")):
            self.side = ops.side_stream()
        self._ev_side = self._ev_main = None
        self._ev_si = self._ev_mi = 0
        if self.side is not None and hasattr(ops, "event"):
            self._ev_side = [ops.event() for _ in range(256)]
            self._ev_main = [ops.event() for _ in range(256)]
        self._alloc()

    def _event(self, side):
        ring = self._ev_side if side else self._ev_main
        if ring is None:
            return None
        if side:
            ev, self._ev_si = ring[self._ev_si], (self._ev_si + 1) % len(ring)
        else:
            ev, self._ev_mi = ring[self._ev_mi], (self._ev_mi + 1) % len(ring)
        return ev

    def _zero(self, t):
        if hasattr(self.ops, "zero_") and t.is_contiguous():
            self.ops.zero_(t)
        else:
            t.zero_()

    def _copy(self, dst, src):
        if (hasattr(self.ops, "copy_") and dst.is_contiguous() and src.is_contiguous() and
                dst.dtype == src.dtype and src.is_cuda and dst.numel() == src.numel()):
            self.ops.copy_(dst, src)
        else:
            dst.copy_(src)

    def _t(self, *shape, f32=False):
        return torch.zeros(*shape, dtype=torch.float32 if f32 else self.dt, device=self.dev)

    def _alloc(self):
# ... 133 lines not shown
        d, s = self.depths, self.s
        out = []
        if net == "G":
            out.append(("first", "first_block.block.0.module", d[0], d[0]))
            for i in range(s):
                out.append((f"a{i}", f"blocks.{i}.block.0.module", d[i + 1], d[i]))
                out.append((f"b{i}", f"blocks.{i}.block.3.module", d[i + 1], d[i + 1]))
        else:
            out.append(("mb", "minibatch_normalization_block.conv.module", d[0], d[0] + 1))
            for i in range(s):
                out.append((f"a{i}", f"blocks.{i}.block.0.module", d[i + 1], d[i + 1]))
                out.append((f"b{i}", f"blocks.{i}.block.2.module", d[i], d[i + 1]))
        return out

    def alloc_packs(self):
        ops = self.ops
        self.packs = {}
        for net in (("G", "D") if self.forward_only is None else (self.forward_only[0],)):
            for key, _, cout, cin in self._conv_list(net):
                nf = ops.packed_elems(L.PACK_FWD, cout, cin)
                nd = ops.packed_elems(L.PACK_DGRAD, cout, cin)
                self.packs[(net, key)] = (
                    torch.empty(nf, dtype=self.dt, device=self.dev),
                    torch.empty(nd, dtype=self.dt, device=self.dev),
                    torch.empty(cout, dtype=torch.float32, device=self.dev),
                    he(cin * 9))

    def pack(self, net, P):
        if not hasattr(self, "packs"):
            self.alloc_packs()
        if hasattr(self, "_packed"):
            self._packed[net] = True
        ops = self.ops
        if hasattr(ops, "pack_table"):
            ents = []
            for key, wname, cout, cin in self._conv_list(net):
                pf, pd, bs, c = self.packs[(net, key)]
                ents.append((P[wname + ".weight"], P[wname + ".bias"], pf, pd, bs, c))
            sig = tuple(t.data_ptr() for e in ents for t in (e[0], e[1]))
            tabs = self.__dict__.setdefault("_pack_tables", {})
            if net not in tabs or tabs[net][0] != sig:
                tabs[net] = (sig, ops.pack_table(ents))
            ops.conv_pack_batch(tabs[net][1])
            return
        for key, wname, cout, cin in self._conv_list(net):
            pf, pd, bs, c = self.packs[(net, key)]
            w = P[wname + ".weight"]
            ops.conv_pack(L.PACK_FWD, w, c, pf)
            ops.conv_pack(L.PACK_DGRAD, w, c, pd)
            ops.blend(c, P[wname + ".bias"], 0.0, None, bs)

    def _conv(self, net, key, x, y, H, cin, cout, flags, aux=None, y2=None, out_scale=1.0,
              dgrad=False, bias=True, xbits=None):
        pf, pd, bs, _ = self.packs[(net, key)]
        if not dgrad and bias:
            flags |= L.CONV_BIAS
        need = self._ws_need("c", H, cin, cout, False)
        kw = dict(xbits=xbits) if xbits is not None else {}
        self.ops.conv3x3(x, pd if dgrad else pf, y, B=self.B, H=H, W=H, cin=cin, cout=cout,
                         flags=flags, slope=SLOPE, out_scale=out_scale,
                         bias=bs if (flags & L.CONV_BIAS) else None, aux=aux, y2=y2,
                         ws=self.ws if need else None, **kw)

    def _ws_bytes(self, kind, H, cin, cout, ups, B=None):
        B = self.B if B is None else B
        key = (kind, H, cin, cout, ups, B)
        need = self._ws_cache.get(key)
        if need is None:
            if kind == "c":
                need = self.ops.conv_workspace_bytes(B=B, H=H, W=H, cin=cin, cout=cout)
            else:
                need = self.ops.wgrad_workspace_bytes(B=B, H=H, W=H, cin=cin, cout=cout,
                                                      ups=ups)
            self._ws_cache[key] = need
        return need

    def _ws_need(self, kind, H, cin, cout, ups, B=None):
        need = self._ws_bytes(kind, H, cin, cout, ups, B)
        if need and (self.ws is None or self.ws.numel() * 4 < need):
            self.ws = torch.empty((need + 3) // 4, dtype=torch.float32, device=self.dev)
        return need

    def _wgrad(self, net, key, x, gz, dW, H, cin, cout, ups=False, db=None, gzbits=None,
               gscale=1.0, main=False):
        c = self.packs[(net, key)][3]
        kw = dict(gzbits=gzbits, slope=SLOPE) if gzbits is not None else {}
        if self.side is None or FORCE_SERIAL or main:
            need = self._ws_need("w", H, cin, cout, ups)
            self.ops.conv_wgrad(x, gz, dW, B=self.B, H=H, W=H, cin=cin, cout=cout, ups=ups,
                                scale=c * gscale, db=db, ws=self.ws if need else None, **kw)
            return
        need = self._ws_bytes("w", H, cin, cout, ups)
        if need and (self.ws_side is None or self.ws_side.numel() * 4 < need):
            self.side.synchronize()
            self.ws_side = torch.empty((need + 3) // 4, dtype=torch.float32, device=self.dev)
        self._side_call((net,), self.ops.conv_wgrad, x, gz, dW, B=self.B, H=H, W=H, cin=cin,
                        cout=cout, ups=ups, scale=c * gscale, db=db,
                        ws=self.ws_side if need else None, **kw)

    def _side_call(self, nets, fn, *a, **kw):
        if self.side is None or FORCE_SERIAL:
            return fn(*a, **kw)
        self._side_wait_main()
        with torch.cuda.stream(self.side):
            fn(*a, **kw)
        ev = self._event(True) or torch.cuda.Event()
        ev.record(self.side)
        for n in nets:
            self._side_ev[n] = ev

    def _side_wait_main(self):
        ev = self._event(False)
        if ev is None:
            self.side.wait_stream(torch.cuda.current_stream())
        else:
            ev.record(torch.cuda.current_stream())
            ev.wait(self.side)

    def _side_join(self, net=None):
        if not self._side_ev:
            return
        keys = list(self._side_ev) if net is None else [net]
        cur = torch.cuda.current_stream()
        for k in keys:
            ev = self._side_ev.pop(k, None)
            if ev is not None:
                if isinstance(ev, torch.cuda.Event):
                    cur.wait_event(ev)
                else:
                    ev.wait(cur)

    def _tail_main_on(self):
        return self.side is not None and not FORCE_SERIAL and self.tail_main

    def _tail_wait(self):
        ev, self._tail_ev = getattr(self, "_tail_ev", None), None
        if ev is not None:
            cur = torch.cuda.current_stream()
            if isinstance(ev, torch.cuda.Event):
                cur.wait_event(ev)
            else:
                ev.wait(cur)

    def _ready_main(self, net, *prefixes):
        if self.grad_ready is None:
            return
        if self.side is not None:
            self._side_wait_main()
        self._ready(net, *prefixes)

    def _conv_sup(self):
        f = getattr(self.ops, "conv_supported", None)
        if f is None:
            return None
        Bs = self._Bs
        return lambda B, **kw: all(f(B=b, **kw) for b in Bs)

    def _dbits(self, i):
        key = ("dbits", i, 0, 0, 0)
        if key not in self._ws_cache:
            f = self._conv_sup()
            d, Ri = self.depths, 8 * 2 ** i
            ok = bool(self.fuse_dbits and f is not None and d[i] % 16 == 0 and
                      Ri >= self.dbits_min_res)
            if ok:
                B = self.B
                ok = (f(B=B, H=Ri, W=Ri, cin=d[i + 1], cout=d[i],
                        flags=L.CONV_BIAS | L.CONV_LRELU | L.CONV_POOL | L.CONV_Y2_BITS)
                      and f(B=B, H=Ri, W=Ri, cin=d[i], cout=d[i + 1],
                            flags=L.CONV_UPS_IN | L.CONV_X_BITS | L.CONV_MASK)
                      and f(B=B, H=Ri, W=Ri, cin=d[i + 1], cout=d[i],
                            flags=L.CONV_MASK | L.CONV_AUX_BITS | L.CONV_POOL)
                      and f(B=B, H=Ri, W=Ri, cin=d[i + 1], cout=d[i], flags=L.CONV_GZ_BITS))
            self._ws_cache[key] = ok
        return self._ws_cache[key]

    def _ubits(self, i):
        key = ("ubits", i, 0, 0, 0)
        if key not in self._ws_cache:
            f = self._conv_sup()
            d, Ri, B = self.depths, 8 * 2 ** i, self.B
            ok = bool(f is not None and self.fuse_dbits and self.fuse_ubits and
                      not self._dbits(i) and d[i] % 16 == 0)
            if ok:
                ok = (f(B=B, H=Ri, W=Ri, cin=d[i + 1], cout=d[i],
                        flags=L.CONV_BIAS | L.CONV_LRELU | L.CONV_POOL | L.CONV_Y2_BITS)
                      and f(B=B, H=Ri, W=Ri, cin=d[i + 1], cout=d[i],
                            flags=L.CONV_MASK | L.CONV_AUX_BITS | L.CONV_POOL))
            self._ws_cache[key] = ok
        return self._ws_cache[key]

    def _rgbbits(self):
        key = ("rgbbits", 0, 0, 0, 0)
        if key not in self._ws_cache:
            f = self._conv_sup()
            d, s, R, B = self.depths, self.s, self.R, self.B
            ok = bool(f is not None and self.fuse_dbits and self.fuse_rgbbits and s >= 1 and
                      d[s] % 8 == 0 and
                      d[s] <= 64 and R >= self.dbits_min_res and
                      f(B=B, H=R, W=R, cin=d[s], cout=d[s], flags=L.CONV_MASK | L.CONV_AUX_BITS))
            self._ws_cache[key] = ok
        return self._ws_cache[key]

    def _rgbw(self):
        key = ("rgbw", 0, 0, 0, 0)
        if key not in self._ws_cache:
            f = self._conv_sup()
            d, s, R, B = self.depths, self.s, self.R, self.B
            ok = bool(self.fuse_rgbw and self._rgbbits() and hasattr(self.ops, "conv3x3_rgbw") and
                      f(B=B, H=R, W=R, cin=d[s], cout=d[s],
                        flags=L.CONV_MASK | L.CONV_AUX_BITS | L.CONV_RGBW))
            self._ws_cache[key] = ok
        return self._ws_cache[key]

    def _rgbd(self):
        key = ("rgbd", 0, 0, 0, 0)
        if key not in self._ws_cache:
            f = self._conv_sup()
            d, s, R, B = self.depths, self.s, self.R, self.B
            ok = bool(self.fuse_rgbd and self._rgbbits() and hasattr(self.ops, "conv3x3_rgbd") and
                      B <= 16 and
                      f(B=B, H=R, W=R, cin=d[s], cout=d[s],
                        flags=L.CONV_MASK | L.CONV_AUX_BITS | L.CONV_RGBD))
            self._ws_cache[key] = ok
        return self._ws_cache[key]

    def _pn_pool(self, i):
        key = ("pnpool", i, 0, 0, 0)
        if key not in self._ws_cache:
            f = getattr(self.ops, "conv_supported", None)
            d, Ri, B = self.depths, 8 * 2 ** i, self.B
            ok = bool(i >= 1 and f is not None and self.fuse_pn_pool and
                      self._pn_fused(Ri // 2, d[i], d[i], L.CONV_LRELU) and
                      f(B=B, H=Ri, W=Ri, cin=d[i + 1], cout=d[i],
                        flags=L.CONV_POOL | L.CONV_PNBWD))
            self._ws_cache[key] = ok
        return self._ws_cache[key]

    def _pn_fused(self, H, cin, cout, flags):
        key = ("pn", H, cin, cout, flags)
        if key not in self._ws_cache:
            f = getattr(self.ops, "conv_supported", None)
            ok = bool(self.fuse_pixnorm and f is not None)
            for b in self._GBs:
                need = self._ws_need("c", H, cin, cout, False, b)
                ok = ok and bool(f(B=b, H=H, W=H, cin=cin, cout=cout,
                                   flags=flags | L.CONV_PIXNORM | L.CONV_BIAS, ws_bytes=need))
            self._ws_cache[key] = ok
        return self._ws_cache[key]

    def _pnb_fused(self, H, cin, cout):
        key = ("pnb", H, cin, cout)
        if key not in self._ws_cache:
            f = getattr(self.ops, "conv_supported", None)
            ok = bool(self.fuse_pixnorm and self.fuse_pnbwd and f is not None and
                      self._pn_fused(H, cin, cout, L.CONV_UPS_IN | L.CONV_LRELU))
            if ok:
                need = self._ws_need("c", H, cout, cout, False)
                ok = bool(f(B=self.B, H=H, W=H, cin=cout, cout=cout, flags=L.CONV_PNBWD,
                            ws_bytes=need))
            self._ws_cache[key] = ok
        return self._ws_cache[key]

    def _g_conv_pn(self, key, x, u, y, r, H, cin, cout, flags, keep):
        if self._pn_fused(H, cin, cout, flags):
            self._conv("G", key, x, y, H, cin, cout, flags | L.CONV_PIXNORM, y2=r if keep else None)
        else:
            self._conv("G", key, x, u, H, cin, cout, flags)
            self.ops.pixnorm(u, y, cout)

    def _g_pn_bwd(self, key, u, y, r, gy, gz, H, cin, cout, flags):
        if self._pn_fused(H, cin, cout, flags):
            self.ops.pixnorm_lrelu_bwd_y(y, r, gy, gz, cout, SLOPE)
        else:
            self.ops.pixnorm_lrelu_bwd(u, gy, gz, cout, SLOPE)

    def g_forward(self, P, z, alpha, keep=True):
        ops, g, d, s, B = self.ops, self.g, self.depths, self.s, self.B
        self._side_join("G")
        if z is not g["z"]:
            self._copy(g["z"], z)
        ops.pixnorm(g["z"], g["zn"], self.latent)
        Wf = P["latent_format_layer.module.weight"]
        ops.linear(g["zn"], Wf, P["latent_format_layer.module.bias"], g["f"], B=B,
                   flags=L.LIN_BIAS | L.LIN_LRELU | L.LIN_OUT_CHW, scale=he(self.latent),
# ... 121 lines not shown
                pn_done = i - 1
            else:
                self._conv("G", f"a{i}", g[f"gza{i}"], g[f"gy{i}"], Ri, d[i + 1], d[i], flags,
                           dgrad=True, out_scale=1.0)
        fb = "first_block.block.0.module."
        self._g_pn_bwd("first", g["u0"], g["y0"], g["r0"], g["gy0"], g["gz0"], 4, d[0], d[0],
                       L.CONV_LRELU)
        tail = self._tail_main_on()
        if not tail:
            self._wgrad("G", "first", g["h0"], g["gz0"], GR[fb + "weight"], 4, d[0], d[0],
                        db=GR[fb + "bias"])
            self._ready("G", fb)
        self._conv("G", "first", g["gz0"], g["gh0"], 4, d[0], d[0], 0, dgrad=True)
        ops.pixnorm_lrelu_bwd(g["f"], g["gh0"], g["gzf"], d[0], self.hyper.slope_cfg)
        lin = (g["zn"], g["gzf"], GR["latent_format_layer.module.weight"],
               GR["latent_format_layer.module.bias"])
        lkw = dict(B=B, flags=L.LIN_OUT_CHW, scale=he(self.latent))
        if tail:
            self._wgrad("G", "first", g["h0"], g["gz0"], GR[fb + "weight"], 4, d[0], d[0],
                        db=GR[fb + "bias"], main=True)
            ops.linear_wgrad(*lin, **lkw)
            self._ready_main("G", fb, "latent_format_layer.module.")
        else:
            self._side_call(("G",), ops.linear_wgrad, *lin, **lkw)
            self._ready("G", "latent_format_layer.module.")

    def d_forward(self, P, img, alpha, join=True):
        ops, D, d, s, B, R = self.ops, self.dd, self.depths, self.s, self.B, self.R
        if join:
            self._side_join("D")
        fr = "fromRGB_blocks.{}.fromRGB.module."
        ops.from_rgb(img, P[fr.format(s) + "weight"], P[fr.format(s) + "bias"], he(3), D["yrgb"],
                     B=B, R=R, C=d[s], down=False, slope=SLOPE,
                     **(dict(ybits=D["rgbb"]) if self._rgbbits() else {}))
        low = self._low(alpha)
        self._last_dlow = low
        if low:
            ops.from_rgb(img, P[fr.format(s - 1) + "weight"], P[fr.format(s - 1) + "bias"], he(3),
                         D["yd"], B=B, R=R // 2, C=d[s - 1], down=True, slope=SLOPE)
        h = D["yrgb"]
        for i in reversed(range(s)):
            Ri = 8 * 2 ** i
            self._conv("D", f"a{i}", h, D[f"a{i}"], Ri, d[i + 1], d[i + 1], L.CONV_LRELU)
            if self._dbits(i):
                self._conv("D", f"b{i}", D[f"a{i}"], D[f"p{i}"], Ri, d[i + 1], d[i],
                           L.CONV_LRELU | L.CONV_POOL | L.CONV_Y2_BITS, y2=D[f"mb{i}"],
                           out_scale=0.25)
            elif self._ubits(i):
                self._conv("D", f"b{i}", D[f"a{i}"], D[f"p{i}"], Ri, d[i + 1], d[i],
                           L.CONV_LRELU | L.CONV_POOL | L.CONV_Y2_BITS, y2=D[f"mb{i}"],
                           out_scale=0.25)
            else:
                self._conv("D", f"b{i}", D[f"a{i}"], D[f"p{i}"], Ri, d[i + 1], d[i],
                           L.CONV_LRELU | L.CONV_POOL, y2=D[f"bf{i}"], out_scale=0.25)
            if i == s - 1 and low:
                ops.blend(1.0 - alpha, D["yd"], alpha, D[f"p{i}"], D["hblend"])
                h = D["hblend"]
            else:
                h = D[f"p{i}"]
        self.h_mb = h
        self.h_mb_key = "yrgb" if s == 0 else ("hblend" if (s == 1 and low) else "p0")
        ops.mbstd_fwd(h, D["m"], B=B, HW=16, C=d[0])
        self._conv("D", "mb", D["m"], D["c"], 4, d[0] + 1, d[0], L.CONV_LRELU)
        mb = "minibatch_normalization_block.linear.module."
        ops.linear(D["c"], P[mb + "weight"], P[mb + "bias"], D["l1"], B=B,
                   flags=L.LIN_BIAS | L.LIN_LRELU | L.LIN_IN_CHW, scale=he(16 * d[0]), slope=SLOPE)
        ops.linear(D["l1"], P["decision_layer.module.weight"], P["decision_layer.module.bias"],
                   D["logit"], B=B, flags=L.LIN_BIAS, scale=he(d[0]))
        if self.trace is not None:
            self.trace("D", self)
        return D["logit"]

    def _ready(self, net, *prefixes):
        if self.grad_ready is None:
            return
        names = [p + k for p in prefixes for k in ("weight", "bias")]
        if self.side is None:
            self.grad_ready(net, names)
            return
        with torch.cuda.stream(self.side):
            self.grad_ready(net, names)

    def d_backward(self, P, GR, u, alpha, img=None, gimg=None, inj_mbstd=None, final=False,
                   gimg_overwrite=False, norms=None, join=True, t_dw=None):
        ops, D, d, s, B, R = self.ops, self.dd, self.depths, self.s, self.B, self.R
        if join:
            self._side_join("D")
        self._tail_ev = self._side_ev.get("D")
        tail = final and GR is not None and self._tail_main_on()
        fr = "fromRGB_blocks.{}.fromRGB.module."
        rgbw = (tail and gimg is None and s >= 1 and isinstance(img, torch.Tensor) and
                self._rgbw())
        rgbd = (GR is None and gimg is not None and gimg_overwrite and s >= 1 and self._rgbd())
        low_a = self._low(alpha)
        self._t_rgb_done = bool(rgbd and t_dw is not None and not low_a)
        ready = (lambda *p: self._ready("D", *p)) if final else (lambda *p: None)
        dec = "decision_layer.module."
        lin = "minibatch_normalization_block.linear.module."
        if GR is not None:
            self._side_call(("D",), ops.linear_wgrad,
                            D["l1"], u, GR[dec + "weight"], GR[dec + "bias"], B=B, flags=0,
                            scale=he(d[0]))
            ready(dec)
        ops.linear_dgrad(u, P[dec + "weight"], D["gzl1"], B=B, flags=L.LIN_MASK, scale=he(d[0]),
                         slope=SLOPE, aux=D["l1"])
        if GR is not None:
            self._side_call(("D",), ops.linear_wgrad,
                            D["c"], D["gzl1"], GR[lin + "weight"], GR[lin + "bias"], B=B,
                            flags=L.LIN_IN_CHW, scale=he(16 * d[0]))
            ready(lin)
        ops.linear_dgrad(D["gzl1"], P[lin + "weight"], D["gzc"], B=B,
                         flags=L.LIN_IN_CHW | L.LIN_MASK, scale=he(16 * d[0]), slope=SLOPE,
                         aux=D["c"])
        if GR is not None:
            cv = "minibatch_normalization_block.conv.module."
            self._wgrad("D", "mb", D["m"], D["gzc"], GR[cv + "weight"], 4, d[0] + 1, d[0],
                        db=GR[cv + "bias"])
            ready(cv)
        self._conv("D", "mb", D["gzc"], D["gm"], 4, d[0], r4(d[0] + 1), 0, dgrad=True)
        ops.mbstd_bwd(self.h_mb, D["gm"], D["gh"], B=B, HW=16, C=d[0])
        if inj_mbstd is not None:
            ops.blend(1.0, D["gh"], 1.0, inj_mbstd, D["gh"])
        g = D["gh"]
        low = self._low(alpha)
        tail_jobs = []
        for i in range(s):
            Ri = 8 * 2 ** i
            a, b = f"blocks.{i}.block.0.module.", f"blocks.{i}.block.2.module."
            if i == s - 1 and low:
                ops.unpool_mask(g, D["yd"], D["gzd"], B=B, H=Ri // 2, W=Ri // 2, C=d[i],
                                scale=1.0 - alpha, slope=SLOPE, ups=False)
            sc = 0.25 * (alpha if i == s - 1 else 1.0)
            in_tail = tail and i >= s - max(1, self.tail_levels)
            tail_b = in_tail and (i < s - 1 or self.tail_b)
            if self._dbits(i):
                wgb = dict(db=GR[b + "bias"], gzbits=D[f"mb{i}"], gscale=sc) if GR is not None else None
                if GR is not None and not tail_b:
                    self._wgrad("D", f"b{i}", D[f"a{i}"], g, GR[b + "weight"], Ri, d[i + 1], d[i],
                                **wgb)
                    ready(b)
                elif tail_b:
                    tail_jobs.append(((-i, 1), (f"b{i}", D[f"a{i}"], g, GR[b + "weight"], Ri,
                                                d[i + 1], d[i]), wgb, b))
                self._conv("D", f"b{i}", g, D[f"gza{i}"], Ri, d[i], d[i + 1],
                           L.CONV_MASK | L.CONV_UPS_IN | L.CONV_X_BITS, aux=D[f"a{i}"],
                           dgrad=True, out_scale=sc, xbits=D[f"mb{i}"])
            else:
                if self._ubits(i):
                    ops.unpool_mask(g, None, D[f"gzb{i}"], B=B, H=Ri, W=Ri, C=d[i], scale=sc,
                                    slope=SLOPE, ups=True, bits=D[f"mb{i}"])
                else:
                    ops.unpool_mask(g, D[f"bf{i}"], D[f"gzb{i}"], B=B, H=Ri, W=Ri, C=d[i], scale=sc,
                                    slope=SLOPE, ups=True)
                wgb = dict(db=GR[b + "bias"]) if GR is not None else None
                if GR is not None and not tail_b:
                    self._wgrad("D", f"b{i}", D[f"a{i}"], D[f"gzb{i}"], GR[b + "weight"], Ri,
                                d[i + 1], d[i], **wgb)
                    ready(b)
                elif tail_b:
                    tail_jobs.append(((-i, 1), (f"b{i}", D[f"a{i}"], D[f"gzb{i}"], GR[b + "weight"],
                                                Ri, d[i + 1], d[i]), wgb, b))
                self._conv("D", f"b{i}", D[f"gzb{i}"], D[f"gza{i}"], Ri, d[i], d[i + 1],
                           L.CONV_MASK, aux=D[f"a{i}"], dgrad=True)
            hin = D["yrgb"] if i == s - 1 else (self._top_out(alpha) if i == s - 2 else D[f"p{i + 1}"])
            top_tail = tail and i == s - 1
            if GR is not None and not in_tail:
                self._wgrad("D", f"a{i}", hin, D[f"gza{i}"], GR[a + "weight"], Ri, d[i + 1],
                            d[i + 1],
                            db=GR[a + "bias"])
                ready(a)
            elif in_tail:
                tail_jobs.append(((-i, 0), (f"a{i}", hin, D[f"gza{i}"], GR[a + "weight"], Ri,
                                            d[i + 1], d[i + 1]), dict(db=GR[a + "bias"]), a))
            if i == s - 1 and rgbd:
                fw = fr.format(s) + "weight"
                ops.conv3x3_rgbd(D[f"gza{i}"], self.packs[("D", f"a{i}")][1], B=B, H=Ri, W=Ri,
                                 cin=d[i + 1], cout=d[i + 1], flags=L.CONV_MASK | L.CONV_AUX_BITS,
                                 slope=SLOPE, aux=D["rgbb"], w_rgb=P[fw], f=he(3), gimg=gimg,
                                 norms=None if low_a else norms,
                                 dw=t_dw if self._t_rgb_done else None, s=he(3) / B)
            elif i == s - 1 and rgbw:
                self._tail_wait()
                fw = fr.format(s)
                ops.conv3x3_rgbw(D[f"gza{i}"], self.packs[("D", f"a{i}")][1], B=B, H=Ri, W=Ri,
                                 cin=d[i + 1], cout=d[i + 1], flags=L.CONV_MASK | L.CONV_AUX_BITS,
                                 slope=SLOPE, aux=D["rgbb"], img=img, s=he(3),
                                 dw=GR[fw + "weight"], db=GR[fw + "bias"])
            elif i == s - 1 and self._rgbbits():
                self._conv("D", f"a{i}", D[f"gza{i}"], D["gzrgb"], Ri, d[i + 1], d[i + 1],
                           L.CONV_MASK | L.CONV_AUX_BITS, aux=D["rgbb"], dgrad=True)
            elif i == s - 1:
                self._conv("D", f"a{i}", D[f"gza{i}"], D["gzrgb"], Ri, d[i + 1], d[i + 1],
                           L.CONV_MASK, aux=D["yrgb"], dgrad=True)
            else:
                self._conv("D", f"a{i}", D[f"gza{i}"], D[f"ghin{i}"], Ri, d[i + 1], d[i + 1], 0,
                           dgrad=True)
                g = D[f"ghin{i}"]
            if top_tail:
                self._tail_wait()
                for _, args, kw, pre in sorted(tail_jobs, key=lambda j: j[0]):
                    self._wgrad("D", *args, main=True, **kw)
                    self._ready_main("D", pre)
        if s == 0:
            ops.unpool_mask(D["gh"], D["yrgb"], D["gzrgb"], B=B, H=4, W=4, C=d[0], scale=1.0,
                            slope=SLOPE, ups=False)
        fr = "fromRGB_blocks.{}.fromRGB.module."
        w = P[fr.format(s) + "weight"]
        if rgbw:
            self._ready_main("D", fr.format(s))
        elif GR is not None and tail and gimg is None:
            self._tail_wait()
            ops.from_rgb_bwd(D["gzrgb"], w, he(3), B=B, R=R, C=d[s], down=False, img=img,
                             dw=GR[fr.format(s) + "weight"], db=GR[fr.format(s) + "bias"])
            self._ready_main("D", fr.format(s))
        elif GR is not None:
            self._side_call(("D", "G"), ops.from_rgb_bwd,
                            D["gzrgb"], w, he(3), B=B, R=R, C=d[s], down=False, img=img,
                            dw=GR[fr.format(s) + "weight"], db=GR[fr.format(s) + "bias"])
            ready(fr.format(s))
        if gimg is not None and not rgbd:
            ops.from_rgb_bwd(D["gzrgb"], w, he(3), B=B, R=R, C=d[s], down=False, gimg=gimg,
                             **self._gimg_kw(gimg_overwrite, None if low else norms))
        if low:
            w1 = P[fr.format(s - 1) + "weight"]
            if GR is not None:
                self._side_call(("D", "G"), ops.from_rgb_bwd,
                                D["gzd"], w1, he(3), B=B, R=R // 2, C=d[s - 1], down=True, img=img,
                                dw=GR[fr.format(s - 1) + "weight"],
                                db=GR[fr.format(s - 1) + "bias"])
                ready(fr.format(s - 1))
            if gimg is not None:
                ops.from_rgb_bwd(D["gzd"], w1, he(3), B=B, R=R // 2, C=d[s - 1], down=True,
                                 gimg=gimg, **self._gimg_kw(False, norms))

    @staticmethod
    def _gimg_kw(overwrite, norms):
        kw = {}
        if overwrite:
            kw["gimg_overwrite"] = True
        if norms is not None:
            kw["norms"] = norms
        return kw

    def _fused_penalty(self):
        return hasattr(self.ops, "penalty_scale")

    def _input_grad(self, P, u, alpha, mode, w=0.0, GR=None):
        ops, D, B = self.ops, self.dd, self.B
        if self._fused_penalty():
            fw = f"fromRGB_blocks.{self.s}.fromRGB.module.weight"
            self.d_backward(P, None, u, alpha, gimg=D["gimg"], gimg_overwrite=True,
                            norms=D["gp_norms"],
                            t_dw=GR[fw] if (GR is not None and mode == "r1") else None)
            ops.penalty_scale(mode, D["gp_norms"], w, self.loss[2:3], D["gp_scale"])
            return L.ImgMix(D["gimg"], a=D["gp_scale"])
        D["gimg"].zero_()
        self.d_backward(P, None, u, alpha, gimg=D["gimg"])
        if mode == "r1":
            ops.r1_penalty(D["gimg"], B, self.loss[2:3], D["gbar"])
        else:
            ops.gp_penalty(D["gimg"], w, self.loss[2:3], D["gp_norms"], D["gbar"])
        return D["gbar"]

    def d_tangent(self, P, GR, gbar, u, alpha):
        ops, D, d, s, B, R = self.ops, self.dd, self.depths, self.s, self.B, self.R
        self._side_join("D")
        fr = "fromRGB_blocks.{}.fromRGB.module."
        mk = dict(mask_bits=D["rgbb"]) if self._rgbbits() else dict(mask_y=D["yrgb"])
        ops.from_rgb(gbar, P[fr.format(s) + "weight"], None, he(3), D["trgb"], B=B, R=R, C=d[s],
                     down=False, slope=SLOPE, **mk)
        if not getattr(self, "_t_rgb_done", False):
            self._side_call(("D",), ops.from_rgb_bwd,
                            D["gzrgb"], P[fr.format(s) + "weight"], he(3), B=B, R=R, C=d[s],
                            down=False, img=gbar, dw=GR[fr.format(s) + "weight"])
        self._t_rgb_done = False
        low = self._low(alpha)
        if low:
            ops.from_rgb(gbar, P[fr.format(s - 1) + "weight"], None, he(3), D["td"], B=B, R=R // 2,
                         C=d[s - 1], down=True, slope=SLOPE, mask_y=D["yd"])
            self._side_call(("D",), ops.from_rgb_bwd,
                            D["gzd"], P[fr.format(s - 1) + "weight"], he(3), B=B, R=R // 2,
                            C=d[s - 1], down=True, img=gbar, dw=GR[fr.format(s - 1) + "weight"])
        t = D["trgb"]
        for i in reversed(range(s)):
            Ri = 8 * 2 ** i
            a, b = f"blocks.{i}.block.0.module.", f"blocks.{i}.block.2.module."
            self._conv("D", f"a{i}", t, D[f"ta{i}"], Ri, d[i + 1], d[i + 1], L.CONV_MASK,
                       aux=D[f"a{i}"], bias=False)
            self._wgrad("D", f"a{i}", t, D[f"gza{i}"], GR[a + "weight"], Ri, d[i + 1], d[i + 1])
            if self._dbits(i):
                self._conv("D", f"b{i}", D[f"ta{i}"], D[f"tp{i}"], Ri, d[i + 1], d[i],
                           L.CONV_MASK | L.CONV_AUX_BITS | L.CONV_POOL, aux=D[f"mb{i}"],
                           bias=False, out_scale=0.25)
                gb1 = D["gh"] if i == 0 else D[f"ghin{i - 1}"]
                self._wgrad("D", f"b{i}", D[f"ta{i}"], gb1, GR[b + "weight"], Ri, d[i + 1], d[i],
                            gzbits=D[f"mb{i}"], gscale=0.25 * (alpha if i == s - 1 else 1.0))
            elif self._ubits(i):
                self._conv("D", f"b{i}", D[f"ta{i}"], D[f"tp{i}"], Ri, d[i + 1], d[i],
                           L.CONV_MASK | L.CONV_AUX_BITS | L.CONV_POOL, aux=D[f"mb{i}"],
                           bias=False, out_scale=0.25)
                self._wgrad("D", f"b{i}", D[f"ta{i}"], D[f"gzb{i}"], GR[b + "weight"], Ri,
                            d[i + 1], d[i])
            else:
                self._conv("D", f"b{i}", D[f"ta{i}"], D[f"tbf{i}"], Ri, d[i + 1], d[i],
                           L.CONV_MASK, aux=D[f"bf{i}"], bias=False)
                self._wgrad("D", f"b{i}", D[f"ta{i}"], D[f"gzb{i}"], GR[b + "weight"], Ri,
                            d[i + 1], d[i])
                ops.avgpool2(D[f"tbf{i}"], D[f"tp{i}"], B=B, H=Ri, W=Ri, C=d[i])
            if i == s - 1 and low:
                ops.blend(1.0 - alpha, D["td"], alpha, D[f"tp{i}"], D["tblend"])
                t = D["tblend"]
            else:
                t = D[f"tp{i}"]
        ops.mbstd_r1(self.h_mb, t, D["gm"], D["tm"], D["inj"], B=B, HW=16, C=d[0])
        cv = "minibatch_normalization_block.conv.module."
        self._conv("D", "mb", D["tm"], D["tc"], 4, d[0] + 1, d[0], L.CONV_MASK, aux=D["c"],
                   bias=False)
        self._wgrad("D", "mb", D["tm"], D["gzc"], GR[cv + "weight"], 4, d[0] + 1, d[0])
        lin = "minibatch_normalization_block.linear.module."
        ops.linear(D["tc"], P[lin + "weight"], None, D["tl1"], B=B,
                   flags=L.LIN_IN_CHW | L.LIN_MASK, scale=he(16 * d[0]), slope=SLOPE, aux=D["l1"])
        self._side_call(("D",), ops.linear_wgrad,
                        D["tc"], D["gzl1"], GR[lin + "weight"], None, B=B, flags=L.LIN_IN_CHW,
                        scale=he(16 * d[0]))
        dec = "decision_layer.module."
        ops.linear(D["tl1"], P[dec + "weight"], None, D["tout"], B=B, flags=0, scale=he(d[0]))
        self._side_call(("D",), ops.linear_wgrad,
                        D["tl1"], u, GR[dec + "weight"], None, B=B, flags=0, scale=he(d[0]))
        return D["tout"], D["inj"]

    def d_step(self, PG, PD, GD, real, z, alpha_G, alpha_D, gp_eps=None, before_fake=None):
        ops, D, B, hp = self.ops, self.dd, self.B, self.hyper
        GD_flat = self._GD_flat
        self._zero(GD_flat)
        self._zero(self.loss[:3])
        self._zero(self.loss[4:5])
        if self._merged():
            return self._d_step_merged(PG, PD, GD, real, z, alpha_G, alpha_D, before_fake, gp_eps)
        if self._low(alpha_D):
            ops.img_fade(real, alpha_D, D["real_in"])
            xr = D["real_in"]
        else:
            xr = real
        if hp.gp_mode == "r1":
            self.d_forward(PD, xr, alpha_D)
            ops.bce(D["logit"], True, 1.0, self.loss[0:1], D["u"], D["hl"])
            gbar = self._input_grad(PD, D["u"], alpha_D, "r1", GR=GD)
            tout, inj = self.d_tangent(PD, GD, gbar, D["u"], alpha_D)
            ops.mul_add(D["u"], tout.view(-1), D["hl"], D["u2"])
            self.d_backward(PD, GD, D["u2"], alpha_D, img=xr, inj_mbstd=inj)
        else:
            self.d_forward(PD, xr, alpha_D)
            ops.bce(D["logit"], True, 1.0, self.loss[0:1], D["u"], None)
            if hp.W_drift:
                ops.drift(D["logit"], hp.W_drift, self.loss[4:5], D["u"])
            self.d_backward(PD, GD, D["u"], alpha_D, img=xr)
        if before_fake is not None:
            before_fake()
        img_fake = self.g_forward(PG, z, alpha_G, keep=False)
        if self.keep_fake_D:
            img_fake = img_fake.clone()
        self.d_forward(PD, img_fake, alpha_D)
        ops.bce(D["logit"], False, 1.0, self.loss[1:2], D["u"], None)
        self.d_backward(PD, GD, D["u"], alpha_D, img=img_fake, final=hp.gp_mode == "r1")
        if hp.gp_mode != "r1":
            self._wgan_gp(PD, GD, xr, img_fake, gp_eps, alpha_D)
        self._side_join()
        return xr, img_fake

    def _merged(self):
        if self.dd2 is None or self.hyper.gp_mode not in ("r1", "wgan-gp"):
            return False
        return self.hyper.gp_mode == "r1" or not hasattr(self._pending_G, "wait")

    @contextlib.contextmanager
    def _pair(self, b2=False):
        saved = (self.dd, self.B)
        self.dd, self.B = (self.dd2b if b2 else self.dd2), 2 * saved[1]
        try:
            yield
        finally:
            self.dd, self.B = saved

    def _d_step_merged(self, PG, PD, GD, real, z, alpha_G, alpha_D, before_fake, gp_eps=None):
        ops, hp = self.ops, self.hyper
        B = self.B
        D1, D2 = self.dd, self.dd2
        X = D2["xin"]
        if hasattr(self._pending_G, "wait") and hp.gp_mode == "r1":
            return self._d_step_merged_b2(PG, PD, GD, real, z, alpha_G, alpha_D, before_fake)
        if before_fake is not None:
            before_fake()
        img_fake = self._g_forward_d_half(PG, z, alpha_G)
        trace, self.trace = self.trace, None
        try:
            if self._low(alpha_D):
                ops.img_fade(real, alpha_D, X[:B])
            else:
                self._copy(X[:B], real)
            with self._pair():
                self.d_forward(PD, X, alpha_D)
        finally:
            self.trace = trace
        h2 = self.h_mb
        self.h_mb = h2[:B]
        if trace is not None:
            trace("D", self)
            self.dd = self.dd_hi
            try:
                trace("D", self)
            finally:
                self.dd = D1
        if hp.gp_mode != "r1":
            ops.bce(D1["logit"], True, 1.0, self.loss[0:1], D1["u"], None)
            if hp.W_drift:
                ops.drift(D1["logit"], hp.W_drift, self.loss[4:5], D1["u"])
            ops.bce(D2["logit"][B:], False, 1.0, self.loss[1:2], D2["u"][B:], None)
            self.h_mb = h2
            try:
                with self._pair(b2=True):
                    self.d_backward(PD, GD, D2["u"], alpha_D, img=X)
            finally:
                self.h_mb = h2[:B]
            self._wgan_gp(PD, GD, X[:B], X[B:], gp_eps, alpha_D)
            self._side_join()
            return X[:B], (img_fake.clone() if self.keep_fake_D else img_fake)
        ops.bce(D1["logit"], True, 1.0, self.loss[0:1], D1["u"], D1["hl"])
        ops.bce(D2["logit"][B:], False, 1.0, self.loss[1:2], D2["u2"][B:], None)
        gbar = self._input_grad(PD, D1["u"], alpha_D, "r1", GR=GD)
        tout, inj = self.d_tangent(PD, GD, gbar, D1["u"], alpha_D)
        ops.mul_add(D1["u"], tout.view(-1), D1["hl"], D1["u2"])
        self.h_mb = h2
        try:
            with self._pair(b2=True):
                self.d_backward(PD, GD, D2["u2"], alpha_D, img=X, inj_mbstd=D2["inj"], final=True,
                                join=not self.sep_b2)
        finally:
            self.h_mb = h2[:B]
        self._side_join()
        return X[:B], (img_fake.clone() if self.keep_fake_D else img_fake)

    def _g_forward_d_half(self, PG, z, alpha_G):
        z_g = self._z_g
        self._z_g = None
        if z_g is None:
            return self.g_forward(PG, z, alpha_G, keep=False)
        B, g2 = self.B, self.g2
        self._copy(g2["z"][:B], z)
        self._copy(g2["z"][B:], z_g)
        trace, self.trace = self.trace, None
        saved = self.g, self.B
        self.g, self.B = g2, 2 * B
        try:
            self.g_forward(PG, g2["z"], alpha_G, keep=True)
        finally:
            self.g, self.B = saved
            self.trace = trace
        self._g_done = True
        if trace is not None:
            trace("G", self)
            self.g = self.g_hi
            try:
                trace("G", self)
            finally:
                self.g = self.g_lo
        return self.g["img"]

    def _d_step_merged_b2(self, PG, PD, GD, real, z, alpha_G, alpha_D, before_fake):
        ops = self.ops
        B = self.B
        D1, D2 = self.dd, self.dd2
        X = D2["xin"]
        if self._low(alpha_D):
            ops.img_fade(real, alpha_D, X[:B])
        else:
            self._copy(X[:B], real)
        self.d_forward(PD, X[:B], alpha_D)
        ops.bce(D1["logit"], True, 1.0, self.loss[0:1], D1["u"], D1["hl"])
        gbar = self._input_grad(PD, D1["u"], alpha_D, "r1", GR=GD)
        tout, inj = self.d_tangent(PD, GD, gbar, D1["u"], alpha_D)
        ops.mul_add(D1["u"], tout.view(-1), D1["hl"], D1["u2"])
        if before_fake is not None:
            before_fake()
        img_fake = self._g_forward_d_half(PG, z, alpha_G)
        self.dd = self.dd_hi
        try:
            self.d_forward(PD, X[B:], alpha_D, join=not self.sep_b2)
        finally:
            self.dd = D1
        ops.bce(D2["logit"][B:], False, 1.0, self.loss[1:2], D2["u2"][B:], None)
        self.h_mb = D2[self.h_mb_key]
        try:
            with self._pair(b2=True):
                self.d_backward(PD, GD, D2["u2"], alpha_D, img=X, inj_mbstd=D2["inj"], final=True,
                                join=not self.sep_b2)
        finally:
            self.h_mb = D1[self.h_mb_key]
        self._side_join()
        return X[:B], (img_fake.clone() if self.keep_fake_D else img_fake)

    def _wgan_gp(self, PD, GD, xr, xf, eps, alpha):
        ops, D, B = self.ops, self.dd, self.B
        D["gp_eps"].copy_(eps)
        if self._fused_penalty():
            torch.sub(D["ones"].view(-1, 1), D["gp_eps"], out=D["gp_c"])
            interp = L.ImgMix(xr, xf, D["gp_eps"], D["gp_c"])
        else:
            ops.gp_interp(xr, xf, D["gp_eps"], D["interp"])
            interp = D["interp"]
        self.d_forward(PD, interp, alpha)
        gbar = self._input_grad(PD, D["ones"], alpha, "wgan-gp", self.hyper.W_gp)
        tout, inj = self.d_tangent(PD, GD, gbar, D["ones"], alpha)
        self.d_backward(PD, GD, D["zeros"], alpha, img=interp, inj_mbstd=inj, final=True)

    def g_step(self, PG, PD, GG, z, alpha_G, alpha_D, before_d=None):
        ops, D, hp = self.ops, self.dd, self.hyper
        self._zero(self._GG_flat)
        self._zero(self.loss[3:4])
        if self._g_done:
            self._g_done = False
            self.g = self.g_hi
            try:
                return self._g_step_rest(PG, PD, GG, self.g["img"], alpha_G, alpha_D, before_d)
            finally:
                self.g = self.g_lo
        img = self.g_forward(PG, z, alpha_G)
        return self._g_step_rest(PG, PD, GG, img, alpha_G, alpha_D, before_d)

    def _g_step_rest(self, PG, PD, GG, img, alpha_G, alpha_D, before_d):
        ops, D, hp = self.ops, self.dd, self.hyper
        if before_d is not None:
            before_d()
        self.d_forward(PD, img, alpha_D)
        ops.bce(D["logit"], True, hp.W_adv, self.loss[3:4], D["u"], None)
        if self._fused_penalty():
            self.d_backward(PD, None, D["u"], alpha_D, gimg=D["gimg"], gimg_overwrite=True)
        else:
            D["gimg"].zero_()
            self.d_backward(PD, None, D["u"], alpha_D, gimg=D["gimg"])
        self.g_backward(PG, GG, D["gimg"], alpha_G)
        self._side_join()
        return img

    def bind(self, fpG: FlatParams, fpD: FlatParams, hyper: Hyper):
        if getattr(self, "fpG", None) is fpG and self.fpD is fpD and self.hyper is hyper:
            return
        if getattr(self, "_pending_G", None) is not None:
            self._finish_G()
        self.fpG, self.fpD, self.hyper = fpG, fpD, hyper
        self._GD_flat, self._GG_flat = fpD.grad, fpG.grad
        self._pending_G = None
        self._packed = {"G": False, "D": False}

    def adam(self, fp: FlatParams, lr):
        hp = self.hyper
        if fp is self.fpG:
            self._side_join("G")
        else:
            self._side_join()
        n = fp.n_live
        if hasattr(self.ops, "adam_dev"):
            if fp._step_dev_host != fp.step:
                fp.step_dev.fill_(fp.step)
            fp.step += 1
            fp._step_dev_host = fp.step
            self.ops.adam_dev(fp.flat[:n], fp.grad[:n], fp.m[:n], fp.v[:n], lr=lr, beta1=hp.beta1,
                              beta2=hp.beta2, eps=hp.eps, step_dev=fp.step_dev)
            return
        fp.step += 1
        self.ops.adam(fp.flat[:n], fp.grad[:n], fp.m[:n], fp.v[:n], lr=lr, beta1=hp.beta1,
                      beta2=hp.beta2, eps=hp.eps, step=fp.step)

    def train_step(self, real, z1, z2, alpha_G, alpha_D, grad_hook=None, gp_eps=None):
        fpG, fpD, hp = self.fpG, self.fpD, self.hyper
        PG, PD = fpG.views, fpD.views
        ov = self.overlap_g_exchange
        if ov < 0:
            ov = int(getattr(getattr(grad_hook, "__self__", None), "world", 2) > 1)
# ... 54 lines not shown
```

Measured before the change: 396.2 images/sec.

## Merge R1 tangent weight-gradient convs into the D backward wgrad as two-segment launches

Adds a two-segment wgrad kernel mode (for both the DMA and the regular bf16 paths) that reads the first B1 images from one activation/gradient pair and the rest from a second pair. The tangent weight-gradient terms from d_tangent are deferred and fused into the matching d_backward wgrad launches, with bias gradients taken only from the second segment. This removes separate wgrad launches and their partial reductions over small batches, which gives better tile occupancy. The cost is extra template instantiations, per-tile segment selection logic and a deferral bookkeeping path that must consume every pending term.

Result: no change. 396.3 images/sec (median of 2 runs) (+0.0%).

```diff
diff --git a/include/pggan_hip.h b/include/pggan_hip.h
--- a/include/pggan_hip.h
+++ b/include/pggan_hip.h
@@ -87,6 +87,11 @@
 int pg_conv3x3_wgrad_ex(int dtype, const pg_conv_desc* d, const void* x, const void* gz,
                         const void* gzbits, float scale, float* dw, float* db, void* ws,
                         size_t ws_bytes, void* stream);
+int pg_conv3x3_wgrad_pair_supported(int dtype, const pg_conv_desc* d, int B1);
+int pg_conv3x3_wgrad_pair(int dtype, const pg_conv_desc* d, int B1, const void* x, const void* gz,
+                          const void* gzbits, const void* x2, const void* gz2, const void* gzbits2,
+                          float scale, float* dw, float* db, void* ws, size_t ws_bytes,
+                          void* stream);
 int pg_bias_grad(int dtype, int npix, int C, int cs, const void* g, float scale, float* db,
                  void* scratch, void* stream);
 
diff --git a/pggan_amd/_lib.py b/pggan_amd/_lib.py
--- a/pggan_amd/_lib.py
+++ b/pggan_amd/_lib.py
@@ -98,6 +98,9 @@
     "pg_conv3x3_wgrad_workspace_size": ([_I, ctypes.POINTER(ConvDesc)], _SZ),
     "pg_conv3x3_wgrad": ([_I, ctypes.POINTER(ConvDesc), _VP, _VP, _F, _VP, _VP, _VP, _SZ, _VP],
                          _I),
+    "pg_conv3x3_wgrad_pair_supported": ([_I, ctypes.POINTER(ConvDesc), _I], _I),
+    "pg_conv3x3_wgrad_pair": ([_I, ctypes.POINTER(ConvDesc), _I, _VP, _VP, _VP, _VP, _VP, _VP, _F,
+                               _VP, _VP, _VP, _SZ, _VP], _I),
     "pg_bias_grad": ([_I, _I, _I, _I, _VP, _F, _VP, _VP, _VP], _I),
     "pg_pixnorm_fwd": ([_I, _I, _I, _I, _VP, _VP, _VP], _I),
     "pg_pixnorm_lrelu_bwd": ([_I, _I, _I, _I, _VP, _VP, _F, _I, _VP, _VP], _I),
@@ -416,13 +419,31 @@
         d = ConvDesc(B, H, W, cin, cout, 0, 0, 0, 0, CONV_UPS_IN if ups else 0, 0.0, 1.0, 0)
         return int(self.lib.pg_conv3x3_wgrad_workspace_size(self.dt, ctypes.byref(d)))
 
+    wgrad_pair = True
+
+    def wgrad_pair_supported(self, *, B, B1, H, W, cin, cout, x_cs, gz_cs, ups=False,
+                             gzb_cs=0):
+        fl = (CONV_UPS_IN if ups else 0) | (CONV_GZ_BITS if gzb_cs else 0)
+        d = ConvDesc(B, H, W, cin, cout, x_cs, gz_cs, 0, 0, fl, 0.2, 1.0, gzb_cs)
+        return bool(self.lib.pg_conv3x3_wgrad_pair_supported(self.dt, ctypes.byref(d), B1))
+
     def conv_wgrad(self, x, gz, dw, *, B, H, W, cin, cout, ups, scale, db=None, ws=None,
-                   gzbits=None, slope=0.2):
-        self._cuda(x, gz, dw, db, ws, gzbits)
+                   gzbits=None, slope=0.2, x2=None, gz2=None, gzbits2=None, B1=None):
+        self._cuda(x, gz, dw, db, ws, gzbits, x2, gz2, gzbits2)
         fl = (CONV_UPS_IN if ups else 0) | (CONV_GZ_BITS if gzbits is not None else 0)
         d = ConvDesc(B, H, W, cin, cout, x.shape[-1], gz.shape[-1], 0, 0, fl, slope, 1.0,
                      gzbits.shape[-1] if gzbits is not None else 0)
         wsb = ws.numel() * ws.element_size() if ws is not None else 0
+        if x2 is not None:
+            if (gz2 is None or B1 is None or (gzbits is None) != (gzbits2 is None) or
+                    x2.shape[-1] != x.shape[-1] or gz2.shape[-1] != gz.shape[-1]):
+                raise ValueError("conv_wgrad: a pair needs x2, gz2, B1 and matching operands")
+            self._chk(self.lib.pg_conv3x3_wgrad_pair(self._dt(gz), ctypes.byref(d), int(B1), _p(x),
+                                                     _p(gz), _p(gzbits), _p(x2), _p(gz2),
+                                                     _p(gzbits2), scale, _p(dw), _p(db), _p(ws),
+                                                     wsb, self._s()),
+                      "conv3x3_wgrad_pair")
+            return
         self._chk(self.lib.pg_conv3x3_wgrad_ex(self._dt(gz), ctypes.byref(d), _p(x), _p(gz),
                                                _p(gzbits), scale, _p(dw), _p(db), _p(ws), wsb,
                                                self._s()),
diff --git a/pggan_amd/csrc/conv.hip b/pggan_amd/csrc/conv.hip
--- a/pggan_amd/csrc/conv.hip
+++ b/pggan_amd/csrc/conv.hip
@@ -762,7 +762,25 @@
   int gzb_cs;
   float slope;
   int xcd_remap;
+  const bf16_t* x2;
+  const bf16_t* gz2;
+  const unsigned char* gzb2;
+  int B1, db_b0;
 };
+
+struct WgPair {
+  const void* x2;
+  const void* gz2;
+  const void* gzbits2;
+  int B1;
+};
+inline void wgb_set_pair(WgBParams& p, const WgPair* pr) {
+  p.x2 = pr ? (const bf16_t*)pr->x2 : p.x;
+  p.gz2 = pr ? (const bf16_t*)pr->gz2 : p.gz;
+  p.gzb2 = pr && p.gzb ? reinterpret_cast<const unsigned char*>(pr->gzbits2) : p.gzb;
+  p.B1 = pr ? pr->B1 : p.B;
+  p.db_b0 = pr ? pr->B1 : 0;
+}
 
 constexpr int WGB_BP = 128;
 constexpr int wgb_maxhalo(int bp) { return bp == 128 ? 288 : 18 * 18; }
@@ -773,7 +791,7 @@
 #ifndef PG_WG_PRE_ALL
 #define PG_WG_PRE_ALL 1
 #endif
-template <int MO, int NC, int WMO, int WNC, int PD, int WPE, bool GZB, int BP>
+template <int MO, int NC, int WMO, int WNC, int PD, int WPE, bool GZB, int BP, bool PAIR = false>
 __global__ __launch_bounds__(256) __attribute__((amdgpu_waves_per_eu(WPE)))
 void wgrad_bf16_kernel(WgBParams p) {
   constexpr bool PRE = PG_WG_PRE_ALL || MO < 4;
@@ -864,23 +882,37 @@
     const bf16_t* gzt = p.gz + (((size_t)b0 * gH + (ty0 >> gs)) * gW + (tx0 >> gs)) * p.gz_cs + o0;
     const unsigned char* gbt =
         gz_bits ? p.gzb + (((size_t)b0 * p.H + ty0) * p.W + tx0) * p.gzb_cs : nullptr;
+    const long long b2 = (long long)b0 - p.B1;
+    const bf16_t* gzt2 = p.gz2 + ((b2 * gH + (ty0 >> gs)) * gW + (tx0 >> gs)) * p.gz_cs + o0;
 #pragma unroll
     for (int k = 0; k < NGZ; ++k) {
       const bool ok = b0 + gznb[k] < p.B;
-      rg[k] = *reinterpret_cast<const u32x4_t*>(ok ? gzt + gzrel[k] : p.gz);
+      if constexpr (PAIR) {
+        static_assert(!GZB, "wgrad_bf16: no two-segment GZ_BITS form");
+        const bool s2 = b0 + gznb[k] >= p.B1;
+        rg[k] = *reinterpret_cast<const u32x4_t*>(ok ? (s2 ? gzt2 : gzt) + gzrel[k] : p.gz);
+        gok |= (ok && s2 ? 0x10000u : 0u) << k;
+      } else {
+        rg[k] = *reinterpret_cast<const u32x4_t*>(ok ? gzt + gzrel[k] : p.gz);
+      }
       if constexpr (gz_bits) rb[k] = *(ok ? gbt + gbrel[k] : p.gzb);
       gok |= (ok ? 1u : 0u) << k;
     }
     const int ys = p.ups ? 1 : 0;
     const bf16_t* xt = PRE ? p.x + c0 + (((size_t)b0 * p.Hin + (ty0 >> ys)) * p.Win + (tx0 >> ys)) * p.x_cs
                               : p.x;
+    const bf16_t* xt2 = p.x2 + c0 + ((b2 * p.Hin + (ty0 >> ys)) * p.Win + (tx0 >> ys)) * p.x_cs;
 #pragma unroll
     for (int k = 0; k < NH; ++k) {
       const int pk = hpk[k];
       const int yy = ty0 + ((pk >> 16) & 0xff) - 1, xx = tx0 + ((pk >> 8) & 0xff) - 1;
       const bool ok = pk >= 0 && b0 + (pk >> 24) < p.B && (unsigned)yy < (unsigned)p.H &&
                       (unsigned)xx < (unsigned)p.W;
-      if constexpr (PRE) {
+      if constexpr (PAIR) {
+        static_assert(!PAIR || PRE, "wgrad_bf16: the two-segment form uses the precomputed offsets");
+        const bool s2 = b0 + (pk >> 24) >= p.B1;
+        rh[k] = *reinterpret_cast<const u32x4_t*>(ok ? (s2 ? xt2 : xt) + hrel[k] : p.x);
+      } else if constexpr (PRE) {
         rh[k] = *reinterpret_cast<const u32x4_t*>(ok ? xt + hrel[k] : p.x);
       } else {
         rh[k] = *reinterpret_cast<const u32x4_t*>(
@@ -910,7 +942,7 @@
         }
       }
       *reinterpret_cast<u32x4_t*>(gzl + grow(pm) + 8 * v) = rg;
-      if (do_db) {
+      if (do_db && (!PAIR || ((gok >> (16 + k)) & 1u))) {
 #pragma unroll
         for (int e = 0; e < 4; ++e) {
           bs[2 * e] += bf_lo(rg[e]);
@@ -1202,12 +1234,14 @@
 
 bool wgrad_dma_ok(const pg_conv_desc* d, const WgbPlan& pl);
 int launch_wgrad_dma(const pg_conv_desc* d, const WgbPlan& pl, const void* x, const void* gz, float scale,
-                     float* dw, float* db, float* ws, size_t ws_bytes, hipStream_t st, const void* gzbits);
-
-template <int MO, int NC, int WMO, int WNC, int PD, int WPE, bool GZB = false, int BP = WGB_BP>
+                     float* dw, float* db, float* ws, size_t ws_bytes, hipStream_t st, const void* gzbits,
+                     const WgPair* pr);
+
+template <int MO, int NC, int WMO, int WNC, int PD, int WPE, bool GZB = false, int BP = WGB_BP,
+          bool PAIR = false>
 int launch_wgrad_bf16(const pg_conv_desc* d, const WgbPlan& pl, const void* x, const void* gz,
                       float scale, float* dw, float* db, float* ws, size_t ws_bytes,
-                      hipStream_t st, const void* gzbits) {
+                      hipStream_t st, const void* gzbits, const WgPair* pr = nullptr) {
   constexpr int BO = WMO * MO * 16, BC = WNC * NC * 16;
   WgBParams p;
   p.x = (const bf16_t*)x; p.gz = (const bf16_t*)gz; p.dw = dw; p.db = db;
@@ -1233,6 +1267,7 @@
   p.gzb_cs = d->xb_cs;
   p.slope = d->slope;
   p.xcd_remap = 1;
+  wgb_set_pair(p, PAIR ? pr : nullptr);
   PG_CHECK_ARG(!p.gzb || (d->xb_cs * 8 >= d->cout && pl.tc.TH % 2 == 0 && pl.tc.TW % 2 == 0),
                "wgrad_bf16: GZ_BITS needs gzbits with >= cout/8 bytes per pixel");
   PG_CHECK_ARG(pl.BP == BP && p.halo_elems <= wgb_maxhalo(BP), "wgrad_bf16: halo %d > %d", p.halo_elems,
@@ -1247,8 +1282,8 @@
   const int need = 4 * 9 * 64 * 4 * 4;
   if (need > lds) lds = need;
   PG_CHECK_ARG(lds <= 160 * 1024, "wgrad_bf16: LDS %d too large", lds);
-  PG_LDS_ATTR((wgrad_bf16_kernel<MO, NC, WMO, WNC, PD, WPE, GZB, BP>), 160 * 1024);
-  PG_KLAUNCH((wgrad_bf16_kernel<MO, NC, WMO, WNC, PD, WPE, GZB, BP>), dim3(pl.ot, pl.ct, pl.splits),
+  PG_LDS_ATTR((wgrad_bf16_kernel<MO, NC, WMO, WNC, PD, WPE, GZB, BP, PAIR>), 160 * 1024);
+  PG_KLAUNCH((wgrad_bf16_kernel<MO, NC, WMO, WNC, PD, WPE, GZB, BP, PAIR>), dim3(pl.ot, pl.ct, pl.splits),
                      dim3(256), lds, st, p);
   PG_LAUNCH_CHECK();
   return wgrad_slab_finish(d, pl, p.mode, ws, dw, db, scale, st);
@@ -1259,9 +1294,16 @@
          (MO == 1 && PD == 2);
 }
 
+bool wgrad_pair_ok(const pg_conv_desc* d, int B1) {
+  if (B1 <= 0 || B1 >= d->B || d->H < 4 || d->W < 4) return false;
+  if (d->cout % 8 || d->x_cs % 8 || d->y_cs % 8) return false;
+  const WgbPlan pl = wgrad_bf16_plan(d);
+  return wgrad_dma_ok(d, pl) || !(d->flags & PG_CONV_GZ_BITS);
+}
+
 int wgrad_bf16_dispatch(const pg_conv_desc* d, const void* x, const void* gz, float scale,
                         float* dw, float* db, float* ws, size_t ws_bytes, hipStream_t st,
-                        const void* gzbits = nullptr) {
+                        const void* gzbits = nullptr, const WgPair* pr = nullptr) {
   PG_CHECK_ARG(!(d->flags & PG_CONV_GZ_BITS) || gzbits, "wgrad_bf16: GZ_BITS without gzbits");
   PG_CHECK_ARG(d->cout % 8 == 0 && d->x_cs % 8 == 0 && d->y_cs % 8 == 0,
                "wgrad_bf16: cout (%d) and channel strides must be multiples of 8", d->cout);
@@ -1270,7 +1312,8 @@
     pl.splits = 1;
     pl.tiles_per_split = pl.ntiles;
   }
-  if (wgrad_dma_ok(d, pl)) return launch_wgrad_dma(d, pl, x, gz, scale, dw, db, ws, ws_bytes, st, gzbits);
+  if (wgrad_dma_ok(d, pl))
+    return launch_wgrad_dma(d, pl, x, gz, scale, dw, db, ws, ws_bytes, st, gzbits, pr);
   const int pd = pl.MO >= 4 ? 4 : 2, wpe = pl.MO >= 4 ? 1 : (pl.MO * pl.WNC >= 2 ? 2 : 3);
   const bool gzb = (d->flags & PG_CONV_GZ_BITS) != 0;
 #define PG_WGB(a, b, c, e, PD, WPE)                                                        \
@@ -1281,6 +1324,9 @@
                                                             ws, ws_bytes, st, gzbits);     \
     }                                                                                      \
     PG_CHECK_ARG(!gzb, "wgrad_bf16: GZ_BITS not instantiated for this tile");              \
+    if (pr)                                                                                \
+      return launch_wgrad_bf16<a, b, c, e, PD, WPE, false, WGB_BP, true>(                  \
+          d, pl, x, gz, scale, dw, db, ws, ws_bytes, st, gzbits, pr);                      \
     return launch_wgrad_bf16<a, b, c, e, PD, WPE, false>(d, pl, x, gz, scale, dw, db, ws,  \
                                                          ws_bytes, st, gzbits);            \
   }
@@ -1801,6 +1847,27 @@
   return PG_OK;
 }
 
+int pg_conv3x3_wgrad_pair_supported(int dtype, const pg_conv_desc* d, int B1) {
+  return (dtype == PG_BF16 && d && wgrad_pair_ok(d, B1)) ? 1 : 0;
+}
+
+int pg_conv3x3_wgrad_pair(int dtype, const pg_conv_desc* d, int B1, const void* x, const void* gz,
+                          const void* gzbits, const void* x2, const void* gz2, const void* gzbits2,
+                          float scale, float* dw, float* db, void* ws, size_t ws_bytes,
+                          void* stream) {
+  PG_CHECK_ARG(d && x && gz && x2 && gz2 && dw, "conv3x3_wgrad_pair: null pointer");
+  const bool gzb = (d->flags & PG_CONV_GZ_BITS) != 0;
+  PG_CHECK_ARG(!gzb || (gzbits && gzbits2), "conv3x3_wgrad_pair: GZ_BITS needs both segments' gzbits");
+  if (dtype != PG_BF16 || !wgrad_pair_ok(d, B1)) {
+    pg_set_error("conv3x3_wgrad_pair: no two-segment kernel for this shape (B1 %d of %d, dtype %d)",
+                 B1, d->B, dtype);
+    return PG_ERR_UNSUPPORTED;
+  }
+  const WgPair pr{x2, gz2, gzbits2, B1};
+  return wgrad_bf16_dispatch(d, x, gz, scale, dw, db, (float*)ws, ws_bytes, (hipStream_t)stream,
+                             gzbits, &pr);
+}
+
 int pg_conv3x3_wgrad_ex(int dtype, const pg_conv_desc* d, const void* x, const void* gz,
                         const void* gzbits, float scale, float* dw, float* db, void* ws,
                         size_t ws_bytes, void* stream) {
diff --git a/pggan_amd/csrc/wgrad_dma.inc b/pggan_amd/csrc/wgrad_dma.inc
--- a/pggan_amd/csrc/wgrad_dma.inc
+++ b/pggan_amd/csrc/wgrad_dma.inc
@@ -42,7 +42,7 @@
                : "=&s"(keep) : "s"(m0v), "v"(voff), "s"(rs) : "memory");
 }
 
-template <int MO, int WNC, bool GZB>
+template <int MO, int WNC, bool GZB, bool PAIR = false>
 __global__ __launch_bounds__(256 * WNC) void wgrad_dma_kernel(WgBParams p) {
 #if defined(__HIP_DEVICE_COMPILE__)
   using G = WgdGeo<MO, WNC, GZB>;
@@ -70,16 +70,23 @@
 
   const unsigned OOB = 0x7fff0000u;
   const int gH = GZB ? p.H >> 1 : p.H, gW = GZB ? p.W >> 1 : p.W;
-  const unsigned gz_nrec = (unsigned)((size_t)p.B * gH * gW * p.gz_cs * 2);
-  const unsigned gzb_nrec = GZB ? (unsigned)((size_t)p.B * p.H * p.W * p.gzb_cs) : 0u;
+  const unsigned gz_ib = (unsigned)(gH * gW * p.gz_cs * 2);
+  const unsigned gzb_ib = GZB ? (unsigned)(p.H * p.W * p.gzb_cs) : 0u;
   constexpr int PPP = 1024 / GRB;
-  const unsigned x_nrec = (unsigned)((size_t)p.B * p.Hin * p.Win * p.x_cs * 2);
+  const unsigned x_ib = (unsigned)(p.Hin * p.Win * p.x_cs * 2);
   const int ys = p.ups ? 1 : 0;
   auto dma_tile = [&](int t, char* base) __attribute__((always_inline)) {
     const int tx0 = (t & (p.tiles_x - 1)) * WGD_TW;
     const int tt = t >> p.lg_tx;
     const int ty0 = (tt & (p.tiles_y - 1)) * WGD_TH;
-    const int b = tt >> p.lg_ty;
+    const int bt = tt >> p.lg_ty;
+    const bool s2 = PAIR && bt >= p.B1;
+    const int b = s2 ? bt - p.B1 : bt;
+    const unsigned nimg = (unsigned)(PAIR ? (s2 ? p.B - p.B1 : p.B1) : p.B);
+    const bf16_t* xs = s2 ? p.x2 : p.x;
+    const bf16_t* gzs = s2 ? p.gz2 : p.gz;
+    const unsigned char* gzbs = s2 ? p.gzb2 : p.gzb;
+    const unsigned gz_nrec = nimg * gz_ib, gzb_nrec = nimg * gzb_ib, x_nrec = nimg * x_ib;
 #pragma unroll
     for (int j = 0; j < G::PPW; ++j) {
       const int k = wid + NW * j;
@@ -90,7 +97,7 @@
         const int py = ty0 + (r >> 4), px = tx0 + (r & 15);
         const int gy = GZB ? py >> 1 : py, gx = GZB ? px >> 1 : px;
         const unsigned v = (unsigned)((((b * gH + gy) * gW + gx) * p.gz_cs + o0 + 8 * s) * 2);
-        hr_dma16(p.gz, gz_nrec, (lds_void_t*)(base + k * 1024), v, 0);
+        hr_dma16(gzs, gz_nrec, (lds_void_t*)(base + k * 1024), v, 0);
         if constexpr (GZB) {
           constexpr int DPP = BO / 32;
           const int pi = lane / DPP;
@@ -100,7 +107,7 @@
             const int qy = ty0 + (r2 >> 4), qx = tx0 + (r2 & 15);
             vb = (unsigned)(((b * p.H + qy) * p.W + qx) * p.gzb_cs + (o0 >> 3) + 4 * (lane % DPP));
           }
-          wgd_dma4(p.gzb, gzb_nrec, (lds_void_t*)(base + G::NPC * 1024 + k * 256), vb);
+          wgd_dma4(gzbs, gzb_nrec, (lds_void_t*)(base + G::NPC * 1024 + k * 256), vb);
         }
       } else {
         constexpr int SPP = HPB / 16;
@@ -111,7 +118,7 @@
         unsigned v = OOB;
         if (P < WGD_HPIX && (unsigned)yy < (unsigned)p.H && (unsigned)xx < (unsigned)p.W)
           v = (unsigned)((((b * p.Hin + (yy >> ys)) * p.Win + (xx >> ys)) * p.x_cs + c0 + 8 * s) * 2);
-        hr_dma16(p.x, x_nrec, (lds_void_t*)(base + k * 1024), v, 0);
+        hr_dma16(xs, x_nrec, (lds_void_t*)(base + k * 1024), v, 0);
       }
     }
   };
@@ -216,7 +223,7 @@
     asm volatile("" ::: "memory");
     if (i + DEPTH < n) dma_tile(t_begin + i + DEPTH, slot(i + DEPTH));
     compute(slot(i));
-    if (do_db) bias_tile(slot(i));
+    if (do_db && (!PAIR || ((t_begin + i) >> (p.lg_tx + p.lg_ty)) >= p.db_b0)) bias_tile(slot(i));
   }
 
   float* red = reinterpret_cast<float*>(smem);
@@ -304,18 +311,25 @@
   return xin <= 0x7fff0000ull && gin <= 0x7fff0000ull && bits <= 0x7fff0000ull && pl.tiles_per_split >= 1;
 }
 
+template <int MO, int WNC, bool GZB, bool PAIR>
+int launch_wgrad_dma_kp(const WgbPlan& pl, const WgBParams& p, hipStream_t st) {
+  using G = WgdGeo<MO, WNC, GZB>;
+  static_assert(G::NTHR * 8 * 4 <= G::LDS && G::LDS <= 160 * 1024, "wgrad_dma: LDS");
+  PG_LDS_ATTR((wgrad_dma_kernel<MO, WNC, GZB, PAIR>), G::LDS);
+  PG_KLAUNCH((wgrad_dma_kernel<MO, WNC, GZB, PAIR>), dim3(pl.ot, pl.ct, pl.splits), dim3(G::NTHR), G::LDS, st, p);
+  PG_LAUNCH_CHECK();
+  return PG_OK;
+}
+
 template <int MO, int WNC, bool GZB = false>
 int launch_wgrad_dma_k(const WgbPlan& pl, const WgBParams& p, hipStream_t st) {
-  using G = WgdGeo<MO, WNC, GZB>;
-  static_assert(G::NTHR * 8 * 4 <= G::LDS && G::LDS <= 160 * 1024, "wgrad_dma: LDS");
-  PG_LDS_ATTR((wgrad_dma_kernel<MO, WNC, GZB>), G::LDS);
-  PG_KLAUNCH((wgrad_dma_kernel<MO, WNC, GZB>), dim3(pl.ot, pl.ct, pl.splits), dim3(G::NTHR), G::LDS, st, p);
-  PG_LAUNCH_CHECK();
-  return PG_OK;
+  return p.B1 < p.B ? launch_wgrad_dma_kp<MO, WNC, GZB, true>(pl, p, st)
+                    : launch_wgrad_dma_kp<MO, WNC, GZB, false>(pl, p, st);
 }
 
 int launch_wgrad_dma(const pg_conv_desc* d, const WgbPlan& pl, const void* x, const void* gz, float scale,
-                     float* dw, float* db, float* ws, size_t ws_bytes, hipStream_t st, const void* gzbits) {
+                     float* dw, float* db, float* ws, size_t ws_bytes, hipStream_t st, const void* gzbits,
+                     const WgPair* pr) {
   WgBParams p{};
   p.x = (const bf16_t*)x; p.gz = (const bf16_t*)gz; p.dw = dw; p.db = db;
   p.B = d->B; p.H = d->H; p.W = d->W;
@@ -329,6 +343,7 @@
   p.gzb_cs = d->xb_cs;
   p.slope = d->slope;
   PG_CHECK_ARG(!gzb || gzbits, "wgrad_dma: GZ_BITS without gzbits");
+  wgb_set_pair(p, pr);
   p.tiles_x = d->W / WGD_TW;
   p.tiles_y = d->H / WGD_TH;
   auto lg2 = [](int v) { int l = 0; while ((1 << l) < v) ++l; return l; };
diff --git a/pggan_amd/engine.py b/pggan_amd/engine.py
--- a/pggan_amd/engine.py
+++ b/pggan_amd/engine.py
@@ -152,6 +152,7 @@
     tail_b=True,
     tail_levels=1,
     fuse_rgbo=False,
+    merge_t_wgrad=0,
 )
 
 
@@ -451,19 +452,26 @@
         return need
 
     def _wgrad(self, net, key, x, gz, dW, H, cin, cout, ups=False, db=None, gzbits=None,
-               gscale=1.0, main=False):
+               gscale=1.0, main=False, pair=None):
         c = self.packs[(net, key)][3]
         kw = dict(gzbits=gzbits, slope=SLOPE) if gzbits is not None else {}
+        B = self.B
+        if pair is not None:
+            x1, gz1, gzbits1 = pair
+            kw.update(x2=x, gz2=gz, B1=x1.shape[0])
+            if gzbits is not None:
+                kw.update(gzbits=gzbits1, gzbits2=gzbits)
+            x, gz, B = x1, gz1, B + x1.shape[0]
         if self.side is None or FORCE_SERIAL or main:
-            need = self._ws_need("w", H, cin, cout, ups)
-            self.ops.conv_wgrad(x, gz, dW, B=self.B, H=H, W=H, cin=cin, cout=cout, ups=ups,
+            need = self._ws_need("w", H, cin, cout, ups, B)
+            self.ops.conv_wgrad(x, gz, dW, B=B, H=H, W=H, cin=cin, cout=cout, ups=ups,
                                 scale=c * gscale, db=db, ws=self.ws if need else None, **kw)
             return
-        need = self._ws_bytes("w", H, cin, cout, ups)
+        need = self._ws_bytes("w", H, cin, cout, ups, B)
         if need and (self.ws_side is None or self.ws_side.numel() * 4 < need):
             self.side.synchronize()
             self.ws_side = torch.empty((need + 3) // 4, dtype=torch.float32, device=self.dev)
-        self._side_call((net,), self.ops.conv_wgrad, x, gz, dW, B=self.B, H=H, W=H, cin=cin,
+        self._side_call((net,), self.ops.conv_wgrad, x, gz, dW, B=B, H=H, W=H, cin=cin,
                         cout=cout, ups=ups, scale=c * gscale, db=db,
                         ws=self.ws_side if need else None, **kw)
 
@@ -570,6 +578,23 @@
                       f(B=B, H=R, W=R, cin=d[s], cout=d[s], flags=L.CONV_MASK | L.CONV_AUX_BITS))
             self._ws_cache[key] = ok
         return self._ws_cache[key]
+
+    def _t_merge(self, key, i, H, cin, cout, x_cs, gz_cs, gzb_cs=0):
+        if not (self.merge_t_wgrad and self.sep_b2 and self.dd2b is not None):
+            return False
+        if self.merge_t_wgrad < 2 and self._tail_main_on() and i >= 0:
+            s = self.s
+            in_tail = i >= s - max(1, self.tail_levels)
+            if in_tail and (key[0] == "a" or i < s - 1 or self.tail_b):
+                return False
+        ck = ("tmerge", key, 0, 0, 0)
+        if ck not in self._ws_cache:
+            f = getattr(self.ops, "wgrad_pair_supported", None)
+            self._ws_cache[ck] = bool(
+                getattr(self.ops, "wgrad_pair", False) and f is not None and
+                f(B=3 * self.B, B1=self.B, H=H, W=H, cin=cin, cout=cout, x_cs=x_cs, gz_cs=gz_cs,
+                  gzb_cs=gzb_cs))
+        return self._ws_cache[ck]
 
     def _rgbw(self):
         key = ("rgbw", 0, 0, 0, 0)
@@ -857,8 +882,10 @@
             self.grad_ready(net, names)
 
     def d_backward(self, P, GR, u, alpha, img=None, gimg=None, inj_mbstd=None, final=False,
-                   gimg_overwrite=False, norms=None, join=True, t_dw=None):
+                   gimg_overwrite=False, norms=None, join=True, t_dw=None, t_pend=None):
         ops, D, d, s, B, R = self.ops, self.dd, self.depths, self.s, self.B, self.R
+        t_pend = dict(t_pend or {})
+        tp = lambda k: dict(pair=t_pend.pop(k)) if k in t_pend else {}
         if join:
             self._side_join("D")
         self._tail_ev = self._side_ev.get("D")
@@ -890,7 +917,7 @@
         if GR is not None:
             cv = "minibatch_normalization_block.conv.module."
             self._wgrad("D", "mb", D["m"], D["gzc"], GR[cv + "weight"], 4, d[0] + 1, d[0],
-                        db=GR[cv + "bias"])
+                        db=GR[cv + "bias"], **tp("mb"))
             ready(cv)
         self._conv("D", "mb", D["gzc"], D["gm"], 4, d[0], r4(d[0] + 1), 0, dgrad=True)
         ops.mbstd_bwd(self.h_mb, D["gm"], D["gh"], B=B, HW=16, C=d[0])
@@ -909,7 +936,8 @@
             in_tail = tail and i >= s - max(1, self.tail_levels)
             tail_b = in_tail and (i < s - 1 or self.tail_b)
             if self._dbits(i):
-                wgb = dict(db=GR[b + "bias"], gzbits=D[f"mb{i}"], gscale=sc) if GR is not None else None
+                wgb = (dict(db=GR[b + "bias"], gzbits=D[f"mb{i}"], gscale=sc, **tp(f"b{i}"))
+                       if GR is not None else None)
                 if GR is not None and not tail_b:
                     self._wgrad("D", f"b{i}", D[f"a{i}"], g, GR[b + "weight"], Ri, d[i + 1], d[i],
                                 **wgb)
@@ -927,7 +955,7 @@
                 else:
                     ops.unpool_mask(g, D[f"bf{i}"], D[f"gzb{i}"], B=B, H=Ri, W=Ri, C=d[i], scale=sc,
                                     slope=SLOPE, ups=True)
-                wgb = dict(db=GR[b + "bias"]) if GR is not None else None
+                wgb = dict(db=GR[b + "bias"], **tp(f"b{i}")) if GR is not None else None
                 if GR is not None and not tail_b:
                     self._wgrad("D", f"b{i}", D[f"a{i}"], D[f"gzb{i}"], GR[b + "weight"], Ri,
                                 d[i + 1], d[i], **wgb)
@@ -942,11 +970,12 @@
             if GR is not None and not in_tail:
                 self._wgrad("D", f"a{i}", hin, D[f"gza{i}"], GR[a + "weight"], Ri, d[i + 1],
                             d[i + 1],
-                            db=GR[a + "bias"])
+                            db=GR[a + "bias"], **tp(f"a{i}"))
                 ready(a)
             elif in_tail:
                 tail_jobs.append(((-i, 0), (f"a{i}", hin, D[f"gza{i}"], GR[a + "weight"], Ri,
-                                            d[i + 1], d[i + 1]), dict(db=GR[a + "bias"]), a))
+                                            d[i + 1], d[i + 1]),
+                                  dict(db=GR[a + "bias"], **tp(f"a{i}")), a))
             if i == s - 1 and rgbd:
                 fw = fr.format(s) + "weight"
                 ops.conv3x3_rgbd(D[f"gza{i}"], self.packs[("D", f"a{i}")][1], B=B, H=Ri, W=Ri,
@@ -976,6 +1005,8 @@
                 for _, args, kw, pre in sorted(tail_jobs, key=lambda j: j[0]):
                     self._wgrad("D", *args, main=True, **kw)
                     self._ready_main("D", pre)
+        if t_pend:
+            raise RuntimeError(f"d_backward: deferred weight terms left over: {sorted(t_pend)}")
         if s == 0:
             ops.unpool_mask(D["gh"], D["yrgb"], D["gzrgb"], B=B, H=4, W=4, C=d[0], scale=1.0,
                             slope=SLOPE, ups=False)
@@ -1037,9 +1068,19 @@
             ops.gp_penalty(D["gimg"], w, self.loss[2:3], D["gp_norms"], D["gbar"])
         return D["gbar"]
 
-    def d_tangent(self, P, GR, gbar, u, alpha):
+    def d_tangent(self, P, GR, gbar, u, alpha, pend=None):
         ops, D, d, s, B, R = self.ops, self.dd, self.depths, self.s, self.B, self.R
         self._side_join("D")
+        defer = pend is not None and not self._low(alpha)
+
+        def wg(key, i, x, gz, dW, H, cin, cout, gzbits=None, **kw):
+            if defer and self._t_merge(key, i, H, cin, cout, x.shape[-1], gz.shape[-1],
+                                       gzbits.shape[-1] if gzbits is not None else 0):
+                pend[key] = (x, gz, gzbits)
+                return
+            if gzbits is not None:
+                kw["gzbits"] = gzbits
+            self._wgrad("D", key, x, gz, dW, H, cin, cout, **kw)
         fr = "fromRGB_blocks.{}.fromRGB.module."
         mk = dict(mask_bits=D["rgbb"]) if self._rgbbits() else dict(mask_y=D["yrgb"])
         ops.from_rgb(gbar, P[fr.format(s) + "weight"], None, he(3), D["trgb"], B=B, R=R, C=d[s],
@@ -1062,25 +1103,23 @@
             a, b = f"blocks.{i}.block.0.module.", f"blocks.{i}.block.2.module."
             self._conv("D", f"a{i}", t, D[f"ta{i}"], Ri, d[i + 1], d[i + 1], L.CONV_MASK,
                        aux=D[f"a{i}"], bias=False)
-            self._wgrad("D", f"a{i}", t, D[f"gza{i}"], GR[a + "weight"], Ri, d[i + 1], d[i + 1])
+            wg(f"a{i}", i, t, D[f"gza{i}"], GR[a + "weight"], Ri, d[i + 1], d[i + 1])
             if self._dbits(i):
                 self._conv("D", f"b{i}", D[f"ta{i}"], D[f"tp{i}"], Ri, d[i + 1], d[i],
                            L.CONV_MASK | L.CONV_AUX_BITS | L.CONV_POOL, aux=D[f"mb{i}"],
                            bias=False, out_scale=0.25)
                 gb1 = D["gh"] if i == 0 else D[f"ghin{i - 1}"]
-                self._wgrad("D", f"b{i}", D[f"ta{i}"], gb1, GR[b + "weight"], Ri, d[i + 1], d[i],
-                            gzbits=D[f"mb{i}"], gscale=0.25 * (alpha if i == s - 1 else 1.0))
+                wg(f"b{i}", i, D[f"ta{i}"], gb1, GR[b + "weight"], Ri, d[i + 1], d[i],
+                   gzbits=D[f"mb{i}"], gscale=0.25 * (alpha if i == s - 1 else 1.0))
             elif self._ubits(i):
                 self._conv("D", f"b{i}", D[f"ta{i}"], D[f"tp{i}"], Ri, d[i + 1], d[i],
                            L.CONV_MASK | L.CONV_AUX_BITS | L.CONV_POOL, aux=D[f"mb{i}"],
                            bias=False, out_scale=0.25)
-                self._wgrad("D", f"b{i}", D[f"ta{i}"], D[f"gzb{i}"], GR[b + "weight"], Ri,
-                            d[i + 1], d[i])
+                wg(f"b{i}", i, D[f"ta{i}"], D[f"gzb{i}"], GR[b + "weight"], Ri, d[i + 1], d[i])
             else:
                 self._conv("D", f"b{i}", D[f"ta{i}"], D[f"tbf{i}"], Ri, d[i + 1], d[i],
                            L.CONV_MASK, aux=D[f"bf{i}"], bias=False)
-                self._wgrad("D", f"b{i}", D[f"ta{i}"], D[f"gzb{i}"], GR[b + "weight"], Ri,
-                            d[i + 1], d[i])
+                wg(f"b{i}", i, D[f"ta{i}"], D[f"gzb{i}"], GR[b + "weight"], Ri, d[i + 1], d[i])
                 ops.avgpool2(D[f"tbf{i}"], D[f"tp{i}"], B=B, H=Ri, W=Ri, C=d[i])
             if i == s - 1 and low:
                 ops.blend(1.0 - alpha, D["td"], alpha, D[f"tp{i}"], D["tblend"])
@@ -1091,7 +1130,7 @@
         cv = "minibatch_normalization_block.conv.module."
         self._conv("D", "mb", D["tm"], D["tc"], 4, d[0] + 1, d[0], L.CONV_MASK, aux=D["c"],
                    bias=False)
-        self._wgrad("D", "mb", D["tm"], D["gzc"], GR[cv + "weight"], 4, d[0] + 1, d[0])
+        wg("mb", -1, D["tm"], D["gzc"], GR[cv + "weight"], 4, d[0] + 1, d[0])
         lin = "minibatch_normalization_block.linear.module."
         ops.linear(D["tc"], P[lin + "weight"], None, D["tl1"], B=B,
                    flags=L.LIN_IN_CHW | L.LIN_MASK, scale=he(16 * d[0]), slope=SLOPE, aux=D["l1"])
@@ -1203,13 +1242,14 @@
         ops.bce(D1["logit"], True, 1.0, self.loss[0:1], D1["u"], D1["hl"])
         ops.bce(D2["logit"][B:], False, 1.0, self.loss[1:2], D2["u2"][B:], None)
         gbar = self._input_grad(PD, D1["u"], alpha_D, "r1", GR=GD)
-        tout, inj = self.d_tangent(PD, GD, gbar, D1["u"], alpha_D)
+        t_pend = {}
+        tout, inj = self.d_tangent(PD, GD, gbar, D1["u"], alpha_D, pend=t_pend)
         ops.mul_add(D1["u"], tout.view(-1), D1["hl"], D1["u2"])
         self.h_mb = h2
         try:
             with self._pair(b2=True):
                 self.d_backward(PD, GD, D2["u2"], alpha_D, img=X, inj_mbstd=D2["inj"], final=True,
-                                join=not self.sep_b2)
+                                join=not self.sep_b2, t_pend=t_pend)
         finally:
             self.h_mb = h2[:B]
         self._side_join()
@@ -1253,7 +1293,8 @@
         self.d_forward(PD, X[:B], alpha_D)
         ops.bce(D1["logit"], True, 1.0, self.loss[0:1], D1["u"], D1["hl"])
         gbar = self._input_grad(PD, D1["u"], alpha_D, "r1", GR=GD)
-        tout, inj = self.d_tangent(PD, GD, gbar, D1["u"], alpha_D)
+        t_pend = {}
+        tout, inj = self.d_tangent(PD, GD, gbar, D1["u"], alpha_D, pend=t_pend)
         ops.mul_add(D1["u"], tout.view(-1), D1["hl"], D1["u2"])
         if before_fake is not None:
             before_fake()
@@ -1268,7 +1309,7 @@
         try:
             with self._pair(b2=True):
                 self.d_backward(PD, GD, D2["u2"], alpha_D, img=X, inj_mbstd=D2["inj"], final=True,
-                                join=not self.sep_b2)
+                                join=not self.sep_b2, t_pend=t_pend)
         finally:
             self.h_mb = D1[self.h_mb_key]
         self._side_join()
```
